# tlemane/kmtricks

Hardware: AMD Instinct MI355X
Metric: k-mers merged/s (merge stage, sum over partitions of input records / time) (higher is better)
Workload: dtype u64 keys / u32 counts (integer)

## Files before the change

### include/kmx.h

```cpp
#ifndef KMX_H
#define KMX_H

#include <stddef.h>
#include <stdint.h>

#ifdef __cplusplus
extern "C" {
#endif

#define KMX_VERSION 2

enum {
  KMX_OK = 0,
  KMX_E_NODEVICE = -1,
  KMX_E_INVAL    = -2,
  KMX_E_NOMEM    = -3,
  KMX_E_HIP      = -4,
  KMX_E_UNSUPPORTED = -5
};

enum {
  KMX_MODE_COUNT = 0,
  KMX_MODE_PA    = 1,
  KMX_MODE_BF    = 2,
  KMX_MODE_BFC   = 3,
  KMX_MODE_BFT   = 4
};

typedef struct kmx_ctx kmx_ctx;

int  kmx_version(void);
int  kmx_device_count(void);
int  kmx_device_memory(int device, uint64_t* free_bytes, uint64_t* total_bytes);
uint64_t kmx_device_warm(int device, uint64_t bytes, const volatile int* stop );
int  kmx_create(int device, kmx_ctx** out);
void kmx_destroy(kmx_ctx* ctx);
const char* kmx_last_error(const kmx_ctx* ctx);
int  kmx_set_profiling(kmx_ctx* ctx, int on);
int  kmx_set_file_order(kmx_ctx* ctx, int on);
void* kmx_stream(kmx_ctx* ctx);


typedef struct {
  const void* recs;
  uint64_t    n;
} kmx_list;

typedef struct {
  uint32_t        n_lists;
  uint32_t        key_words;
  const kmx_list* lists;
  const uint32_t* soft_min;
  uint32_t        rec_min;
  uint32_t        share_min;
  uint32_t        mode;
  uint32_t        bitw;
  uint64_t        lower, upper;
  uint64_t        rows_hint;
  const uint8_t*  list_on_device;
} kmx_merge_task;

#define KMX_STATS_ROWS 6

typedef struct kmx_merge_result kmx_merge_result;

int kmx_merge_dev(kmx_ctx* ctx, const kmx_merge_task* tasks, uint32_t n_tasks, kmx_merge_result** out);
int      kmx_result_wait(kmx_merge_result* r);
double   kmx_result_kernel_ms(kmx_merge_result* r);
int      kmx_result_kernel_parts_ms(kmx_merge_result* r, double* first_ms, double* second_ms);
const char* kmx_result_kernel(const kmx_merge_result* r);
double   kmx_result_transpose_ms(kmx_merge_result* r);
const void* kmx_result_body_dev(kmx_merge_result* r, uint32_t task);
int kmx_result_prepare_body(kmx_merge_result* r, uint32_t task);
uint64_t kmx_result_rows(const kmx_merge_result* r, uint32_t task);
uint64_t kmx_result_sparse_rows(const kmx_merge_result* r, uint32_t task);
uint64_t kmx_result_row_bytes(const kmx_merge_result* r, uint32_t task);
uint64_t kmx_result_body_bytes(const kmx_merge_result* r, uint32_t task);
uint64_t kmx_result_algo_bytes(const kmx_merge_result* r, uint32_t task);
int kmx_result_copy_body(kmx_merge_result* r, uint32_t task, void* host_dst, uint64_t dst_bytes);
int kmx_result_arena(kmx_merge_result* r, uint32_t task, const void** dev_arena, uint64_t* arena_rows);
int kmx_result_copy_order(kmx_merge_result* r, uint32_t task, uint32_t* host_order);
int kmx_result_copy_body_dev(kmx_merge_result* r, uint32_t task, void* dev_dst, uint64_t dst_bytes);
int kmx_result_copy_stats(kmx_merge_result* r, uint32_t task, uint64_t* host_stats );
void kmx_result_free(kmx_merge_result* r);

int kmx_merge_host(kmx_ctx* ctx, const kmx_merge_task* tasks, uint32_t n_tasks, kmx_merge_result** out);
void* kmx_alloc_pinned(size_t bytes);
void  kmx_free_pinned(void* p);

int kmx_merge(kmx_ctx* ctx, const kmx_merge_task* task, void** body, uint64_t* body_bytes,
              uint64_t* rows, uint64_t* stats);


#define KMX_FILTER_M 1u
#define KMX_FILTER_V 2u
#define KMX_FILTER_K 4u
typedef struct {
  uint32_t    key_words;
  uint32_t    mode;
  uint32_t    n_cols;
  uint32_t    want;
  const void* rows;
  uint64_t    n_rows;
  kmx_list    key;
  uint8_t*    marks;
  uint32_t    key_on_device;
} kmx_filter_task;

typedef struct kmx_filter_result kmx_filter_result;

uint8_t* kmx_filter_marks_alloc(kmx_ctx* ctx, uint64_t n);
void     kmx_filter_marks_free(kmx_ctx* ctx, uint8_t* marks);

int kmx_filter_dev(kmx_ctx* ctx, const kmx_filter_task* task, kmx_filter_result** out);
int kmx_filter_host(kmx_ctx* ctx, const kmx_filter_task* task, kmx_filter_result** out);
int      kmx_filter_result_wait(kmx_filter_result* r);
uint64_t kmx_filter_result_rows(kmx_filter_result* r);
uint64_t kmx_filter_result_row_bytes(const kmx_filter_result* r);
uint64_t kmx_filter_result_body_bytes(kmx_filter_result* r);
const void* kmx_filter_result_body_dev(kmx_filter_result* r);
int      kmx_filter_result_copy_body(kmx_filter_result* r, void* host_dst, uint64_t dst_bytes);
uint64_t kmx_filter_result_vector_len(const kmx_filter_result* r);
const void* kmx_filter_result_vector_dev(kmx_filter_result* r);
int      kmx_filter_result_copy_vector(kmx_filter_result* r, uint32_t* host_dst, uint64_t dst_entries);
uint64_t kmx_filter_result_absent(kmx_filter_result* r);
const void* kmx_filter_result_absent_dev(kmx_filter_result* r);
int      kmx_filter_result_copy_absent(kmx_filter_result* r, void* host_dst, uint64_t dst_bytes);
double   kmx_filter_result_kernel_ms(kmx_filter_result* r);
uint64_t kmx_filter_result_algo_bytes(kmx_filter_result* r);
void     kmx_filter_result_free(kmx_filter_result* r);


#define KMX_COMBINE_DROP_LAST 1u
#define KMX_COMBINE_MAX_BLOCKS 64u
typedef struct {
  const void* rows;
  uint64_t    n_rows;
  uint32_t    n_cols;
  uint32_t    count_bytes;
} kmx_block;
typedef struct {
  uint32_t key_words, mode, n_blocks, flags;
  const kmx_block* blocks;
  const uint8_t*   block_on_device;
} kmx_combine_task;

typedef struct kmx_combine_result kmx_combine_result;

int kmx_combine_dev(kmx_ctx* ctx, const kmx_combine_task* task, kmx_combine_result** out);
int kmx_combine_host(kmx_ctx* ctx, const kmx_combine_task* task, kmx_combine_result** out);
int      kmx_combine_result_wait(kmx_combine_result* r);
uint64_t kmx_combine_result_rows(kmx_combine_result* r);
uint64_t kmx_combine_result_row_bytes(const kmx_combine_result* r);
uint64_t kmx_combine_result_body_bytes(kmx_combine_result* r);
const void* kmx_combine_result_body_dev(kmx_combine_result* r);
int      kmx_combine_result_copy_body(kmx_combine_result* r, void* host_dst, uint64_t dst_bytes);
double   kmx_combine_result_kernel_ms(kmx_combine_result* r);
uint64_t kmx_combine_result_algo_bytes(kmx_combine_result* r);
void     kmx_combine_result_free(kmx_combine_result* r);


typedef struct {
  const char*     bases;
  const uint64_t* offsets;
  uint64_t        n_seqs;
  uint32_t        kmer_size, minim_size;
  const uint16_t* repart;
  uint32_t        nb_parts;
  uint32_t        n_cols;
  uint64_t        window;
  const uint8_t* const* rows;
  uint32_t*       hits;
} kmx_query_task;

typedef struct kmx_query_result kmx_query_result;

int kmx_query_dev(kmx_ctx* ctx, const kmx_query_task* task, kmx_query_result** out);
int kmx_query_host(kmx_ctx* ctx, const kmx_query_task* task, kmx_query_result** out);
int      kmx_query_result_wait(kmx_query_result* r);
uint64_t kmx_query_result_n_seqs(const kmx_query_result* r);
int      kmx_query_result_copy_kmers(kmx_query_result* r, uint32_t* host_dst, uint64_t dst_entries);
int      kmx_query_result_copy_hits(kmx_query_result* r, uint32_t* host_dst, uint64_t dst_entries);
uint32_t* kmx_query_result_hits_dev(kmx_query_result* r);
double   kmx_query_result_kernel_ms(kmx_query_result* r);
uint64_t kmx_query_result_algo_bytes(kmx_query_result* r);
void     kmx_query_result_free(kmx_query_result* r);


typedef struct {
  const char*     bases;
  const uint64_t* offsets;
  uint64_t        n_seqs;
  uint32_t        kmer_size, minim_size;
  const uint16_t* repart;
  uint32_t        nb_parts;
  uint32_t        n_cols;
  uint32_t        key_words;
  uint32_t        mode;
  const uint64_t* n_rows;
  const uint8_t* const* rows;
  uint32_t*       hits;
  uint64_t*       sums;
  uint32_t        want_sums;
} kmx_kquery_task;

typedef struct kmx_kquery_result kmx_kquery_result;

int kmx_kquery_dev(kmx_ctx* ctx, const kmx_kquery_task* task, kmx_kquery_result** out);
int kmx_kquery_host(kmx_ctx* ctx, const kmx_kquery_task* task, kmx_kquery_result** out);
int      kmx_kquery_result_wait(kmx_kquery_result* r);
uint64_t kmx_kquery_result_n_seqs(const kmx_kquery_result* r);
int      kmx_kquery_result_copy_kmers(kmx_kquery_result* r, uint32_t* host_dst, uint64_t dst_entries);
int      kmx_kquery_result_copy_hits(kmx_kquery_result* r, uint32_t* host_dst, uint64_t dst_entries);
int      kmx_kquery_result_copy_sums(kmx_kquery_result* r, uint64_t* host_dst, uint64_t dst_entries);
uint32_t* kmx_kquery_result_hits_dev(kmx_kquery_result* r);
uint64_t* kmx_kquery_result_sums_dev(kmx_kquery_result* r);
double   kmx_kquery_result_kernel_ms(kmx_kquery_result* r);
uint64_t kmx_kquery_result_algo_bytes(kmx_kquery_result* r);
void     kmx_kquery_result_free(kmx_kquery_result* r);


typedef struct {
// ... 121 lines not shown
```

### kmtricks_amd/csrc/kmx_api.hip

```cpp
#include "kmx_host.hpp"

#include <algorithm>
#include <chrono>
#include <cmath>
#include <sys/mman.h>
#include <unordered_map>
#include <mutex>
#include <cstdlib>
#include <cstring>
#include <memory>

using namespace kmx;

static thread_local std::string g_create_err;

void* kmx_ctx::dalloc(size_t bytes)
{
  if (bytes == 0) bytes = 256;
  if (bytes >= (8u << 20)) { size_t p2 = (size_t)1 << 23; while (p2 * 2 <= bytes) p2 *= 2; const size_t q = p2 >> 3; bytes = (bytes + q - 1) / q * q; }
  int best = -1;
  for (size_t i = 0; i < pool.size(); i++)
    if (!pool[i].used && pool[i].bytes >= bytes && pool[i].bytes <= 2 * bytes + (1u << 20) &&
        (best < 0 || pool[i].bytes < pool[best].bytes)) best = (int)i;
  if (best >= 0) { pool[best].used = true; return pool[best].p; }
// ... 226 lines not shown
  size_t cap = std::max(bytes, chunk_bytes);
  void* p = nullptr;
  const auto t0 = std::chrono::steady_clock::now();
  hipError_t e = hipMalloc(&p, cap);
  if (e != hipSuccess && cap > bytes) { cap = bytes; e = hipMalloc(&p, cap); }
  { static const bool trace = getenv("KMX_TRACE") != nullptr; if (trace) fprintf(stderr, "[kmx alloc] store chunk %zu MB: %.2f ms\n", cap >> 20, std::chrono::duration<double, std::milli>(std::chrono::steady_clock::now() - t0).count()); }
  if (cur >= 0 && cur != device) (void)hipSetDevice(cur);
  if (e != hipSuccess) return nullptr;
  chunks.push_back({(u8*)p, cap, bytes});
  used += bytes;
  return p;
}
void* kmx_store::try_reserve(size_t bytes)
{
  bytes = (bytes + 255) / 256 * 256;
  if (bytes == 0) bytes = 256;
  std::lock_guard<std::mutex> lk(mu);
  start_ahead();
  if (resvs.size() >= 8 || (limit && used + bytes > limit)) return nullptr;
  for (int pass = 0; pass < 2; pass++) {
    for (size_t i = 0; i < chunks.size(); i++) {
      auto& c = chunks[i];
      if (!chunk_reserved(i) && c.cap - c.fill >= bytes) { resvs.push_back({(int)i, c.fill, bytes}); void* p = c.p + c.fill; c.fill += bytes; used += bytes; return p; }
    }
    if (pass) break;
    { Chunk sp; if (take_spare(bytes, sp)) { chunks.push_back(sp); continue; } }
    int cur = -1; (void)hipGetDevice(&cur);
    if (cur != device && hipSetDevice(device) != hipSuccess) return nullptr;
    const size_t cap = std::max(bytes, chunk_bytes);
    void* p = nullptr;
    const hipError_t e = hipMalloc(&p, cap);
    if (cur >= 0 && cur != device) (void)hipSetDevice(cur);
    if (e != hipSuccess) { (void)hipGetLastError(); return nullptr; }
    chunks.push_back({(u8*)p, cap, 0});
  }
  return nullptr;
}
void kmx_store::commit(void* p, size_t used_bytes)
{
  used_bytes = (used_bytes + 255) / 256 * 256;
  std::lock_guard<std::mutex> lk(mu);
  for (size_t j = 0; j < resvs.size(); j++) {
    const Resv r = resvs[j];
    if (chunks[r.chunk].p + r.off != (u8*)p) continue;
    if (used_bytes > r.bytes) used_bytes = r.bytes;
    chunks[r.chunk].fill = r.off + used_bytes;
    used -= r.bytes - used_bytes;
    resvs.erase(resvs.begin() + j);
    return;
  }
}
extern "C" int kmx_store_create(int device, uint64_t limit_bytes, kmx_store** out)
{
  if (!out) return KMX_E_INVAL;
  *out = nullptr;
  int n = 0;
  if (hipGetDeviceCount(&n) != hipSuccess || n <= 0) { g_create_err = "kmx_store_create: no HIP device; libkmx has no CPU fallback"; return KMX_E_NODEVICE; }
  if (device < 0 || device >= n) { g_create_err = "kmx_store_create: device index out of range"; return KMX_E_INVAL; }
  int cur = -1; (void)hipGetDevice(&cur);
  if (hipSetDevice(device) != hipSuccess) { g_create_err = "kmx_store_create: hipSetDevice failed"; return KMX_E_NODEVICE; }
  size_t fr = 0, tot = 0;
  (void)hipMemGetInfo(&fr, &tot);
  if (cur >= 0 && cur != device) (void)hipSetDevice(cur);
  kmx_store* s = new kmx_store();
  s->device = device;
  s->limit = limit_bytes ? (size_t)limit_bytes : (size_t)(tot / 10 * 6);
  s->chunk_bytes = (size_t)256 << 20;
  { const char* e = getenv("KMX_STORE_CHUNK_MB"); if (e && atol(e) >= 16 && atol(e) <= 65536) s->chunk_bytes = (size_t)atol(e) << 20; }
  *out = s;
  return KMX_OK;
}
extern "C" void kmx_store_destroy(kmx_store* s)
{
  if (!s) return;
  int cur = -1; (void)hipGetDevice(&cur);
  (void)hipSetDevice(s->device);
  (void)hipDeviceSynchronize();
  { std::lock_guard<std::mutex> lk(s->mu); s->stop = true; }
  s->cv.notify_all();
  if (s->ahead.joinable()) s->ahead.join();
  for (auto& c : s->spare) (void)hipFree(c.p);
  for (auto& c : s->chunks) (void)hipFree(c.p);
  if (cur >= 0 && cur != s->device) (void)hipSetDevice(cur);
  delete s;
}
namespace {
std::mutex g_peer_mutex;
signed char g_peer[64][64];
}
int kmx_peer_path(int from, int to)
{
  if (from == to) return 1;
  if (from < 0 || to < 0 || from >= 64 || to >= 64) return 0;
  std::lock_guard<std::mutex> lk(g_peer_mutex);
  if (g_peer[from][to] == 0) {
    int can = 0, cur = -1;
    (void)hipGetDevice(&cur);
    signed char st = -1;
    if (hipDeviceCanAccessPeer(&can, from, to) == hipSuccess && can && hipSetDevice(from) == hipSuccess) {
      const hipError_t e = hipDeviceEnablePeerAccess(to, 0);
      if (e == hipSuccess || e == hipErrorPeerAccessAlreadyEnabled) st = 1;
      (void)hipGetLastError();
    }
    if (cur >= 0) (void)hipSetDevice(cur);
    g_peer[from][to] = st;
    if (getenv("KMX_TRACE")) fprintf(stderr, "[kmx] GPU %d -> GPU %d: %s\n", from, to, st == 1 ? "peer access enabled (copies go over xGMI)" : "no peer access (copies are staged through host memory)");
  }
  return g_peer[from][to] == 1 ? 1 : 0;
}
extern "C" int kmx_peer_access(int from_device, int to_device)
{
  int n = 0;
  if (hipGetDeviceCount(&n) != hipSuccess || from_device < 0 || to_device < 0 || from_device >= n || to_device >= n) return KMX_E_INVAL;
  return kmx_peer_path(from_device, to_device);
}
extern "C" uint64_t kmx_store_used(const kmx_store* s) { return s ? s->used : 0; }
extern "C" uint64_t kmx_store_limit(const kmx_store* s) { return s ? s->limit : 0; }
extern "C" int kmx_copy_to_host(kmx_ctx* ctx, void* dst, const void* src, uint64_t bytes)
{
  if (!ctx) return KMX_E_INVAL;
  if (!bytes) return KMX_OK;
  if (!dst || !src) return ctx->fail(KMX_E_INVAL, "kmx_copy_to_host: null pointer");
  KMX_HIP(ctx, hipSetDevice(ctx->device));
  KMX_HIP(ctx, hipMemcpyAsync(dst, src, bytes, hipMemcpyDeviceToHost, ctx->copy));
  KMX_HIP(ctx, hipStreamSynchronize(ctx->copy));
  return KMX_OK;
}

extern "C" int kmx_copy_to_host_async(kmx_ctx* ctx, void* dst, const void* src, uint64_t bytes, uint32_t* ticket)
{
  if (!ctx) return KMX_E_INVAL;
  if (!ticket || (bytes && (!dst || !src))) return ctx->fail(KMX_E_INVAL, "kmx_copy_to_host_async: null pointer");
  int slot = -1;
  for (int i = 0; i < 8; i++) if (!ctx->copy_out[i]) { slot = i; break; }
  if (slot < 0) return ctx->fail(KMX_E_INVAL, "kmx_copy_to_host_async: KMX_COPIES_AHEAD tickets are out already");
  KMX_HIP(ctx, hipSetDevice(ctx->device));
  if (!ctx->copy_ev[slot]) KMX_HIP(ctx, hipEventCreateWithFlags(&ctx->copy_ev[slot], hipEventDisableTiming));
  if (bytes) KMX_HIP(ctx, hipMemcpyAsync(dst, src, bytes, hipMemcpyDeviceToHost, ctx->copy));
  KMX_HIP(ctx, hipEventRecord(ctx->copy_ev[slot], ctx->copy));
  ctx->copy_out[slot] = true;
  *ticket = (uint32_t)slot;
  return KMX_OK;
}
extern "C" int kmx_copy_wait(kmx_ctx* ctx, uint32_t ticket)
{
  if (!ctx) return KMX_E_INVAL;
  if (ticket >= 8 || !ctx->copy_out[ticket]) return ctx->fail(KMX_E_INVAL, "kmx_copy_wait: no such ticket");
  ctx->copy_out[ticket] = false;
  KMX_HIP(ctx, hipEventSynchronize(ctx->copy_ev[ticket]));
  return KMX_OK;
}

extern "C" int kmx_set_profiling(kmx_ctx* ctx, int on) { if (!ctx) return KMX_E_INVAL; ctx->profiling = on != 0; return KMX_OK; }
extern "C" int kmx_set_file_order(kmx_ctx* ctx, int on) { if (!ctx) return KMX_E_INVAL; ctx->file_order = on != 0; return KMX_OK; }

struct TaskHost {
  u32 N = 0, kw = 1, mode = 0, bitw = 0, c = 1, wl = 0, pivot = 0, rt = 0;
  u32 rec_min = 0, share_min = 0, row_bytes = 0, seg_cap = 0;
  u64 lower = 0, upper = 0, total_recs = 0, out_cap_rows = 0, rows_guess = 0;
  u64 arena_rows = 0;
  bool rows_overflow = false;
  std::vector<u32> len;
  size_t o_recs = 0, o_len = 0, o_smin = 0, o_bounds = 0, o_stats = 0, o_ctrl = 0, o_segs = 0;
  u8* d_out = nullptr; size_t out_bytes = 0;
  u16* d_rowrec = nullptr;
  u32 bft_c = 1;
  u8* d_img = nullptr; size_t img_bytes = 0;
  u64 t_rows = 0, t_cols = 0;
  Seg* d_segs = nullptr;
  Seg* d_segs_own = nullptr;
  u64 rows = 0, nsegs = 0;
  bool done = false;
  bool handed_back = false;
  u32 nblk = 0, nb = 0, rt_cols = 0, slots_cap = 0;
  size_t o_skel = 0, o_nskel = 0, o_rbounds = 0;
  u8* d_ov = nullptr;
  size_t o_spdir = 0;
  size_t o_ovx = 0; u32 xcap = 0;
  u64 sparse_rows = 0;
  u8* d_body = nullptr;
  bool body_ready = false;
  hipEvent_t ev_body = nullptr;
  void* d_body_tmp = nullptr;
  u8* d_dense = nullptr; u32 dpitch = 0, dense_cap = 0; size_t o_gbase = 0;
  u8* d_narrow = nullptr; u32 npitch = 0;
  u64 row_keys = 0;
  bool ordered = false;
  std::vector<u32> src;
  int kernel = 0;
};

struct kmx_merge_result {
  kmx_ctx* ctx = nullptr;
  std::vector<TaskHost> tasks;
  u8* d_meta = nullptr; size_t meta_bytes = 0;
  u8* h_meta = nullptr;
  size_t o_tasks = 0, o_items = 0, o_ticket = 0, o_ctrl0 = 0;
  u32 n_items = 0, grid = 0, max_n = 0, max_c = 0;
  int bf_lds = 0;
  bool is_bf = false, is_bft = false, waited = false;
  bool cols_ext = false, slices_full = false;
  bool cols_resc = false;
  bool share_fix = false;
  bool cols_ord = false;
  bool back_other = false;
  bool rows_small = false;
  bool cols_narrow = false;
  bool rerun_rows = false;
  bool pivot_auto = false;
  bool use_pivot = false;
  bool use_cols = false, cols_auto = false, can_pivot = false, auto_sel = false;
  bool divergent = false;
  u32 given = 0;
  std::vector<TaskHost> subs;
  size_t o_subtasks = 0, o_subitems = 0, o_cols = 0, o_citems = 0;
  u32 n_subitems = 0, n_citems = 0, sub_grid = 0, cols_grid = 0, sub_max_c = 0, sub_max_n = 0, items_grid = 0;
  int status = KMX_OK;
  hipEvent_t ev0 = nullptr, ev1 = nullptr;
  hipEvent_t ev_mid = nullptr;
  hipEvent_t ev2 = nullptr;
  u8* d_in = nullptr;
  u64* d_rem = nullptr; u32 rem_cap = 0;
  bool bft_two_walks = false;
  hipEvent_t ev_in = nullptr;
  u64* d_hctrl = nullptr;
  hipEvent_t ev_pre = nullptr;
  hipEvent_t ev_up = nullptr;
  hipEvent_t ev_done = nullptr;
};

static size_t align_up(size_t x, size_t a) { return (x + a - 1) / a * a; }

static u32 cols_row_lists(u32 rec_min)
{
  for (u32 S = std::max<u32>(8, rec_min + 2); S <= 32; S++) {
    const u32 m = S - rec_min + 1;
    double p = 1.0;
    for (u32 i = 0; i < m; i++) p *= (double)(S - i) / (double)(i + 1) * 0.035;
    if (p < 2e-9) return S;
  }
  return 0;
}

__global__ void k_ctrl_mirror(const u64* __restrict__ src, u64* __restrict__ dst, u32 n)
{
  const u32 i = blockIdx.x * blockDim.x + threadIdx.x;
  if (i < n) dst[i] = src[i];
  __threadfence_system();
}
static int mirror_and_mark(kmx_merge_result* R);
__global__ void k_share_fix(const TaskDev* __restrict__ tasks, u32 kw);

static int launch_batch(kmx_merge_result* R, bool with_bounds)
{
  kmx_ctx* ctx = R->ctx;
  const TaskDev* d_tasks = reinterpret_cast<const TaskDev*>(R->d_meta + R->o_tasks);
  const uint2* d_items = reinterpret_cast<const uint2*>(R->d_meta + R->o_items);
  u32* d_ticket = reinterpret_cast<u32*>(R->d_meta + R->o_ticket);
  const int kw = (int)R->tasks[0].kw, mode = (int)R->tasks[0].mode;
  const ColsOps& CO = cols_ops(kw);
  const u32 nt = (u32)R->tasks.size();
  if (!R->use_cols) KMX_HIP(ctx, hipMemsetAsync(d_ticket, 0, 16, ctx->stream));
  if (ctx->profiling && !R->ev0) { KMX_HIP(ctx, hipEventCreate(&R->ev0)); KMX_HIP(ctx, hipEventCreate(&R->ev1)); }
  if (R->is_bf) {
    if (with_bounds && !R->is_bft) KMX_HIP(ctx, launch_range_bounds_bf(d_tasks, nt, R->max_n, R->max_c, ctx->stream));
    if (R->ev0) KMX_HIP(ctx, hipEventRecord(R->ev0, ctx->stream));
    if (R->is_bft) {
      u32 rt_max = 0; bool rec_bits = true, any_share = false;
      for (auto& H : R->tasks) { rt_max = std::max(rt_max, H.rt); rec_bits = rec_bits && std::max(H.rec_min, H.share_min) <= 1u; any_share = any_share || H.share_min > 0; }
      const u32 bgrid = std::min(R->n_items, (u32)ctx->n_cu * 2u);
      static const bool two_walks_env = getenv("KMX_BFT_TWO_WALKS") != nullptr;
      if (rec_bits && any_share && !R->bft_two_walks && !two_walks_env && !R->d_rem) {
        u64 per_tile = 0;
        for (auto& H : R->tasks) { const u64 tiles = std::max<u64>(1, ((H.upper - H.lower + 1) + H.rt - 1) / H.rt); per_tile = std::max(per_tile, H.total_recs / tiles); }
        u64 cap = std::max<u64>(4096, per_tile / 4);
        cap = std::min<u64>(cap, ((1ull << 30) / 8) / std::max(1u, bgrid));
        R->rem_cap = (u32)cap;
        R->d_rem = (u64*)ctx->dalloc((size_t)bgrid * cap * 8);
      }
      const bool one_walk = R->d_rem && !R->bft_two_walks;
      bool wide = false;
      for (auto& H : R->tasks) { const double m = (double)H.total_recs / H.N * (double)H.rt / (double)(H.upper - H.lower + 1); wide = wide || m + 2.6 * std::sqrt(m) + 8 > (double)bft_round_records(false); }
      KMX_HIP(ctx, launch_merge_bft(d_tasks, d_items, R->n_items, d_ticket, bgrid, R->max_n, rt_max, rec_bits, wide, one_walk ? R->d_rem : nullptr, R->rem_cap, ctx->stream));
    } else
    KMX_HIP(ctx, launch_merge_bf(mode == KMX_MODE_BFC, d_tasks, d_items, R->n_items, d_ticket, R->grid, R->bf_lds, ctx->stream));
  } else if (R->use_cols) {
    const TaskDev* d_subs = reinterpret_cast<const TaskDev*>(R->d_meta + R->o_subtasks);
    const uint2* d_subitems = reinterpret_cast<const uint2*>(R->d_meta + R->o_subitems);
    const ColsDev* d_cols = reinterpret_cast<const ColsDev*>(R->d_meta + R->o_cols);
    const uint2* d_citems = reinterpret_cast<const uint2*>(R->d_meta + R->o_citems);
    static const bool overlap = getenv("KMX_COLS_PREP_OVERLAP") != nullptr;
    hipStream_t ps = overlap ? ctx->aux : ctx->stream;
    if (!R->ev_pre) KMX_HIP(ctx, hipEventCreateWithFlags(&R->ev_pre, hipEventDisableTiming));
    if (overlap && ctx->stream_shared) {
      KMX_HIP(ctx, hipEventRecord(R->ev_pre, ctx->stream));
      KMX_HIP(ctx, hipStreamWaitEvent(ctx->aux, R->ev_pre, 0));
    }
    if (!overlap) KMX_HIP(ctx, hipStreamWaitEvent(ctx->stream, R->ev_up, 0));
    KMX_HIP(ctx, launch_range_bounds(kw, d_subs, nt, R->sub_max_n, R->sub_max_c, ps));
    KMX_HIP(ctx, CO.skel(d_subs, d_subitems, R->n_subitems, ps));
    KMX_HIP(ctx, CO.prep(d_tasks, d_subs, d_cols, nt, ps));
    KMX_HIP(ctx, hipEventRecord(R->ev_pre, ps));
    KMX_HIP(ctx, hipStreamWaitEvent(ctx->stream, R->ev_up, 0));
    KMX_HIP(ctx, launch_range_bounds(kw, d_tasks, nt, R->max_n, R->max_c, ctx->stream));
    KMX_HIP(ctx, hipStreamWaitEvent(ctx->stream, R->ev_pre, 0));
    if (R->ev0) KMX_HIP(ctx, hipEventRecord(R->ev0, ctx->stream));
    const u32 cols_grid_env = getenv("KMX_COLS_GRID") ? (u32)atoi(getenv("KMX_COLS_GRID")) : 0u;
    const u32 sparse_cus_env = getenv("KMX_SPARSE_CUS") ? (u32)atoi(getenv("KMX_SPARSE_CUS")) : 0u;
    KMX_HIP(ctx, CO.merge(mode, (R->cols_ext ? 1 : 0) | (R->cols_resc ? 2 : 0) | (R->cols_ord ? 4 : 0) | (R->cols_narrow ? 8 : 0), d_tasks, d_cols, d_citems, R->n_citems, d_ticket,
                          cols_grid_env ? std::min(cols_grid_env, R->cols_grid) : R->cols_grid, ctx->stream));
    if (R->ev0) { if (!R->ev_mid) KMX_HIP(ctx, hipEventCreate(&R->ev_mid)); KMX_HIP(ctx, hipEventRecord(R->ev_mid, ctx->stream)); }
    KMX_HIP(ctx, CO.sparse(mode | (R->cols_resc ? 2 : 0) | (R->cols_ord ? 4 : 0), d_tasks, d_cols, d_items, R->n_items, nt, d_ticket, sparse_cus_env ? std::min(sparse_cus_env, (u32)ctx->n_cu) : (u32)ctx->n_cu, ctx->stream));
    if (R->share_fix) {
      if ((size_t)R->max_n * 4 > 48 * 1024) KMX_HIP(ctx, hipFuncSetAttribute(reinterpret_cast<const void*>(&k_share_fix), hipFuncAttributeMaxDynamicSharedMemorySize, (int)std::min<size_t>((size_t)R->max_n * 4, 160 * 1024)));
      hipLaunchKernelGGL(k_share_fix, dim3((unsigned)ctx->n_cu * 2u, nt), dim3(256), (size_t)R->max_n * 4, ctx->stream, (const TaskDev*)d_tasks, kw);
      KMX_HIP(ctx, hipGetLastError());
    }
    if (R->ev0) KMX_HIP(ctx, hipEventRecord(R->ev1, ctx->stream));
    return mirror_and_mark(R);
  } else {
    if (with_bounds) KMX_HIP(ctx, launch_range_bounds(kw, d_tasks, nt, R->max_n, R->max_c, ctx->stream));
    if (R->ev0) KMX_HIP(ctx, hipEventRecord(R->ev0, ctx->stream));
    if (R->use_pivot) KMX_HIP(ctx, launch_merge_pivot(kw, mode, d_tasks, d_items, R->n_items, d_ticket, R->grid, ctx->stream));
    else if (R->rows_small) KMX_HIP(ctx, launch_merge_rows_s(kw, mode, d_tasks, d_items, R->n_items, d_ticket, R->grid, R->max_n, ctx->stream));
    else KMX_HIP(ctx, launch_merge_rows(kw, mode, d_tasks, d_items, R->n_items, d_ticket, R->grid, R->max_n, ctx->stream));
  }
  if (R->ev0) KMX_HIP(ctx, hipEventRecord(R->ev1, ctx->stream));
  return mirror_and_mark(R);
}

__global__ __launch_bounds__(256)
void k_share_fix(const TaskDev* __restrict__ tasks, u32 kw)
{
  extern __shared__ u32 sm_s[];
  const TaskDev& T = tasks[blockIdx.y];
  if (T.mode != KMX_MODE_COUNT || T.share_min <= max(1u, T.rec_min)) return;
  if (T.ctrl[2] & (u64)(ERR_FALLBACK | ERR_ROWS_OVERFLOW)) return;
  const u64 rows = T.ctrl[0];
  const u32 lane = threadIdx.x & 63u, N = T.N;
  for (u32 l = threadIdx.x; l < N; l += 256) sm_s[l] = T.soft_min[l];
  __syncthreads();
  const u64 nw = (u64)gridDim.x * 4u;
  for (u64 r = (u64)blockIdx.x * 4u + (threadIdx.x >> 6); r < rows; r += nw) {
    u32* const cnt = reinterpret_cast<u32*>(T.out + r * T.row_bytes + 8u * kw);
    u32 solid = 0, weak = 0;
    for (u32 l0 = 0; l0 < N; l0 += 64u * 16u) {
      u32 c[16];
#pragma unroll
      for (int j = 0; j < 16; j++) { const u32 l = l0 + 64u * j + lane; c[j] = l < N ? cnt[l] : 0u; }
#pragma unroll
      for (int j = 0; j < 16; j++) { const u32 l = l0 + 64u * j + lane; if (c[j]) { if (c[j] >= sm_s[l]) solid++; else weak++; } }
    }
#pragma unroll
    for (int o = 32; o > 0; o >>= 1) { solid += (u32)__shfl_xor((int)solid, o); weak += (u32)__shfl_xor((int)weak, o); }
    if (solid >= T.share_min || !weak) continue;
    for (u32 l = lane; l < N; l += 64) {
      const u32 c = cnt[l];
      if (c && c < sm_s[l]) {
        cnt[l] = 0;
        atomicAdd(reinterpret_cast<unsigned long long*>(&T.stats[(u64)N + l]), ~0ULL);
        atomicAdd(reinterpret_cast<unsigned long long*>(&T.stats[5ull * N + l]), 0ULL - (unsigned long long)c);
      }
    }
  }
}

static int mirror_and_mark(kmx_merge_result* R)
{
  kmx_ctx* ctx = R->ctx;
  if (!R->d_hctrl) {
    void* dp = nullptr;
    KMX_HIP(ctx, hipHostGetDevicePointer(&dp, R->h_meta + R->o_ctrl0, 0));
    R->d_hctrl = reinterpret_cast<u64*>(dp);
  }
  const u32 n = (u32)R->tasks.size() * 8;
  hipLaunchKernelGGL(k_ctrl_mirror, dim3((n + 255) / 256), dim3(256), 0, ctx->stream,
                     reinterpret_cast<const u64*>(R->d_meta + R->o_ctrl0), R->d_hctrl, n);
  KMX_HIP(ctx, hipGetLastError());
  if (!R->ev_done) KMX_HIP(ctx, hipEventCreateWithFlags(&R->ev_done, hipEventDisableTiming));
  KMX_HIP(ctx, hipEventRecord(R->ev_done, ctx->stream));
  return KMX_OK;
}

extern "C" int kmx_merge_dev(kmx_ctx* ctx, const kmx_merge_task* tasks, uint32_t n_tasks, kmx_merge_result** out)
{
  if (!ctx) return KMX_E_INVAL;
  if (!tasks || !n_tasks || !out) return ctx->fail(KMX_E_INVAL, "kmx_merge_dev: null argument");
  *out = nullptr;
  KMX_HIP(ctx, hipSetDevice(ctx->device));
  const u32 kw = tasks[0].key_words, mode = tasks[0].mode;
  if (kw < 1 || kw > 4) return ctx->fail(KMX_E_INVAL, "key_words must be 1 ... 4");
  if (mode > KMX_MODE_BFT) return ctx->fail(KMX_E_INVAL, "unknown mode");
  const bool is_bft = mode == KMX_MODE_BFT;
  const bool is_bf = mode == KMX_MODE_BF || mode == KMX_MODE_BFC || is_bft;
  const ColsOps& CO = cols_ops((int)kw);
  if (is_bf && kw != 1) return ctx->fail(KMX_E_INVAL, "BF/BFC modes take hash keys (key_words = 1)");

  std::unique_ptr<kmx_merge_result> R(new kmx_merge_result());
  R->ctx = ctx; R->is_bf = is_bf; R->is_bft = is_bft;
  R->tasks.resize(n_tasks);
  u64 grand_total = 0;
  {
    u32 mxn0 = 0; for (u32 t = 0; t < n_tasks; t++) mxn0 = std::max(mxn0, tasks[t].n_lists);
    const char* e = getenv("KMX_ROWS_SMALL");
    R->rows_small = !is_bf && kw <= 2 && mxn0 <= 256 && !(e && e[0] == '0');
  }
  const bool rsm = R->rows_small;
  for (u32 t = 0; t < n_tasks; t++) {
    const kmx_merge_task& K = tasks[t];
    TaskHost& H = R->tasks[t];
    if (K.key_words != kw || K.mode != mode) return ctx->fail(KMX_E_INVAL, "all tasks of a batch must share key_words and mode");
    if (K.n_lists == 0 || !K.lists || !K.soft_min) return ctx->fail(KMX_E_INVAL, "task without lists / soft_min");
    H.N = K.n_lists; H.kw = kw; H.mode = mode; H.bitw = K.bitw;
    H.rec_min = K.rec_min; H.share_min = K.share_min; H.lower = K.lower; H.upper = K.upper;
    if (!is_bf && H.N > (u32)rows_cap((int)kw, ~0u)) return ctx->fail(KMX_E_UNSUPPORTED, "more than " + std::to_string(rows_cap((int)kw, ~0u)) + " lists per merge task (COUNT/PA) not supported yet");
    H.len.resize(H.N);
    u32 pivot = 0;
    for (u32 i = 0; i < H.N; i++) {
      if (K.lists[i].n > 0xFFFFFFF0ULL) return ctx->fail(KMX_E_UNSUPPORTED, "list longer than 2^32 records");
      if (K.lists[i].n && !K.lists[i].recs) return ctx->fail(KMX_E_INVAL, "null record pointer");
      if (((uintptr_t)K.lists[i].recs) & 3u) return ctx->fail(KMX_E_INVAL, "record pointers must be 4-byte aligned");
      H.len[i] = (u32)K.lists[i].n;
      H.total_recs += K.lists[i].n;
      if (H.len[i] > H.len[pivot]) pivot = i;
    }
    const u32 longest = H.len[pivot];
    if (H.N >= 5) {
      u32 cand[5] = {0, H.N / 4, H.N / 2, (3 * H.N) / 4, H.N - 1};
      std::sort(cand, cand + 5, [&](u32 a, u32 b) { return H.len[a] < H.len[b]; });
      if (H.len[cand[2]] > 0) pivot = cand[2];
    }
    H.pivot = pivot;
    grand_total += H.total_recs;
    if (is_bf) {
      if (K.upper < K.lower) return ctx->fail(KMX_E_INVAL, "BF window upper < lower");
      if (mode == KMX_MODE_BFC && (K.bitw == 0 || K.bitw > 32)) return ctx->fail(KMX_E_INVAL, "bitw must be in 1..32");
      H.row_bytes = mode != KMX_MODE_BFC ? (H.N + 7) / 8 : (u32)(((u64)H.N * K.bitw + 7) / 8);
      u32 rt = (40960u / H.row_bytes) & ~63u; if (rt < 64) rt = 64;
      if (!is_bft && (u64)rt * H.row_bytes > 96 * 1024) return ctx->fail(KMX_E_UNSUPPORTED, "BF row too wide for one LDS tile");
      H.rt = is_bft ? bft_tile_rows(K.rec_min, K.share_min) : rt;
      H.out_bytes = (size_t)((K.upper - K.lower + 1) * H.row_bytes);
      if (is_bft && H.N > bft_max_lists()) return ctx->fail(KMX_E_UNSUPPORTED, "more than " + std::to_string(bft_max_lists()) + " samples per hash:bft task not supported");
      if (is_bft) {
        H.t_rows = (K.upper - K.lower + 1 + 7) & ~7ULL; H.t_cols = (u64)H.row_bytes * 8;
        H.img_bytes = 0;
        H.nblk = (u32)((H.t_cols + bft_block_lists() - 1) / bft_block_lists());
        H.out_bytes = (size_t)(H.t_cols * (H.t_rows >> 3));
      }
    } else {
      H.row_bytes = kw * 8 + (mode == KMX_MODE_COUNT ? 4 * H.N : (H.N + 7) / 8);
      u32 wl = 0; while (wl < 6 && (H.N << (wl + 1)) <= (u32)(rsm ? rows_s_cap((int)kw, H.N) : rows_cap((int)kw, H.N))) wl++;
      H.wl = wl;
      if (H.row_bytes > (rsm ? rows_s_image_bytes((int)kw) : rows_image_bytes((int)kw))) return ctx->fail(KMX_E_UNSUPPORTED, "row wider than the LDS row image");
      u64 guess = K.rows_hint ? K.rows_hint : 2ULL * longest + 4096;
      if (ctx->rows_per_longest > 0.0) guess = std::max<u64>(guess, (u64)(ctx->rows_per_longest * 1.125 * (double)longest) + 4096);
      if (guess > H.total_recs) guess = H.total_recs;
      H.rows_guess = std::max<u64>(guess, 1);
    }
  }
  if (is_bft) {
    bool all1 = true; u64 wsum = 0;
    for (auto& H : R->tasks) { all1 = all1 && std::max(H.rec_min, H.share_min) <= 1u; wsum += H.upper - H.lower + 1; }
    u32 mxn = 0; for (auto& H : R->tasks) mxn = std::max(mxn, H.N);
// ... 2030 lines not shown
```

### kmtricks_amd/csrc/kmx_host.hpp

```cpp
#pragma once
#include <hip/hip_runtime.h>
#include <string>
#include <functional>
#include <vector>
#include "kmx_dev.hpp"
#include "skf.hpp"
#include "../../include/kmx.h"

namespace kmx {

int rows_lds_bytes(int kw, u32 n_lists);
int rows_cap(int kw, u32 n_lists);
int rows_wgs_per_cu(int kw);
u32 rows_chunk_rows(u32 row_bytes);
u32 rows_image_bytes(int kw);
hipError_t launch_range_bounds(int kw, const TaskDev* tasks, u32 n_tasks, u32 max_n, u32 max_c, hipStream_t st);
hipError_t launch_merge_rows(int kw, int mode, const TaskDev* tasks, const uint2* items, u32 n_items, u32* ticket,
                             u32 grid_x, u32 max_n, hipStream_t st);
int rows_s_cap(int kw, u32 n_lists);
int rows_s_wgs_per_cu(int kw);
u32 rows_s_image_bytes(int kw);
hipError_t launch_merge_rows_s(int kw, int mode, const TaskDev* tasks, const uint2* items, u32 n_items, u32* ticket, u32 grid_x, u32 max_n, hipStream_t st);
int pivot_lds_bytes(int kw);
u32 pivot_max_lists();
hipError_t launch_merge_pivot(int kw, int mode, const TaskDev* tasks, const uint2* items, u32 n_items, u32* ticket,
                              u32 grid_x, hipStream_t st);
struct ColsOps {
  int (*lds_bytes)();
  u32 (*block_lists)();
  u32 (*wgs_per_cu)();
  u32 (*tile_rows)(u32 nb);
  u64 (*scratch_keys)(u32 slots, u32 nblk);
  u64 (*scratch_counts)(u32 slots, u32 nblk);
  u64 (*ext_entries)(u32 slots, u32 nblk);
  u32 (*skel_cap)();
  hipError_t (*skel)(const TaskDev* subs, const uint2* items, u32 n_items, hipStream_t st);
  hipError_t (*prep)(const TaskDev* tasks, const TaskDev* subs, const ColsDev* cols, u32 n_tasks, hipStream_t st);
  hipError_t (*merge)(int mode, int ext, const TaskDev* tasks, const ColsDev* cols, const uint2* items, u32 n_items, u32* ticket, u32 grid_x, hipStream_t st);
  hipError_t (*sparse)(int mode, const TaskDev* tasks, const ColsDev* cols, const uint2* range_items, u32 n_items, u32 n_tasks, u32* ticket, u32 n_cu, hipStream_t st);
  u64 (*dir_bytes)(u32 slots);
  u32 (*groups)(u32 slots);
  hipError_t (*offsets)(const ColsDev* cols, u32 task, u64* goff, hipStream_t st);
  hipError_t (*gather)(const TaskDev* tasks, const ColsDev* cols, u32 task, u32 n_groups, const u64* goff, u8* body, hipStream_t st);
  hipError_t (*order)(const TaskDev* tasks, const ColsDev* cols, u32 task, u32 n_groups, const u64* goff, u32* order, hipStream_t st);
  void (*dbg_dump)();
  void (*phase_prof_dump)();
  u32 key_words;
};
const ColsOps& cols_ops_k1();
const ColsOps& cols_ops_k2();
inline const ColsOps& cols_ops(int kw) { return kw == 2 ? cols_ops_k2() : cols_ops_k1(); }
int bf_lds_bytes(u32 rt, u32 nb, u32 n_lists);
hipError_t launch_range_bounds_bf(const TaskDev* tasks, u32 n_tasks, u32 max_n, u32 max_c, hipStream_t st);
hipError_t launch_merge_bf(int bfc, const TaskDev* tasks, const uint2* items, u32 n_items, u32* ticket,
                           u32 grid_x, int lds, hipStream_t st);
u32 bft_tile_rows(u32 rec_min, u32 share_min);
u32 bft_block_lists();
u32 bft_max_lists();
u32 bft_round_records(bool wide);
u32 bft_fit_rows(u32 max_n, bool bits);
hipError_t launch_merge_bft(const TaskDev* tasks, const uint2* items, u32 n_items, u32* ticket, u32 grid_x, u32 max_n, u32 rt_max, bool rec_bits, bool wide, u64* rem, u32 rem_cap, hipStream_t st);
hipError_t launch_bit_transpose(const u8* in, u8* out, u64 nrows, u64 ncols, hipStream_t st);
u32 filter_tiles(u32 n);
hipError_t launch_filter_match(int kw, const u8* rows, u32 n_rows, u64 irb, const u8* key, u32 n_key, int pa,
                               u32* hit, u32* vec, u8* marks, u32* tile_cnt, hipStream_t st);
hipError_t launch_filter_scan(u32* a, u32 n, hipStream_t st);
hipError_t launch_filter_move(const u8* rows, u32 n_rows, u64 irb, u64 orb, const u32* hit, const u32* vec, const u32* tile_base,
                              u8* out, hipStream_t st);
hipError_t launch_filter_absent_count(const u8* marks, u32 n_key, u32* tile_cnt, hipStream_t st);
hipError_t launch_filter_absent_scatter(int kw, const u8* key, const u8* marks, u32 n_key, const u32* tile_base, u8* out, hipStream_t st);
struct CombineBlock {
  const u8* rows;
  u64 irb;
  u64 key_off;
  u32 n_rows, n_cols;
  u32 cb;
  u32 pos;
  u32 toff;
  u32 ntiles;
};
u32 combine_tiles(u32 n);
hipError_t launch_combine_keys(int kw, const CombineBlock* blocks, u32 nb, u32 n_slots, u64* keys, hipStream_t st);
hipError_t launch_combine_first(int kw, const CombineBlock* blocks, u32 nb, u32 n_slots, const u64* keys, u32* tcnt, u64* fbits, hipStream_t st);
hipError_t launch_combine_scan(const CombineBlock* blocks, u32 nb, u32* tcnt, hipStream_t st);
hipError_t launch_combine_place(int kw, const CombineBlock* blocks, u32 nb, u32 n_slots, const u64* keys, u32* tcnt, u64* fbits, u32* src, u64 cap, hipStream_t st);
hipError_t launch_combine_total(const CombineBlock* blocks, u32 nb, const u32* tcnt, const u32* src, u64 cap, int drop_last, u32* tot, hipStream_t st);
hipError_t launch_combine_move(int pa, const CombineBlock* blocks, u32 nb, u32 kb, u32 n_cols, u32 orb, const u32* src, u64 cap, const u32* tot,
                               u8* out, hipStream_t st);
void query_chunks(u64 n_bases, u32 n_parts, u32* n_tiles, u32* n_chunks, u32* tiles_per_chunk);
hipError_t launch_query_keys(int kw, const char* bases, const u64* offsets, u32 n_seqs, u64 n_bases, int k, int m, const u16* repart, u64 window,
                             u32 n_tiles, u32 n_chunks, u32 tiles_per_chunk, u64* keys, u32* hist , u32* n_kmers , hipStream_t st);
hipError_t launch_query_parts(const u32* cell, u32 n_parts, u32 n_chunks, u32* pstart , hipStream_t st);
hipError_t launch_query_scatter(const u64* keys, const u64* offsets, u32 n_seqs, u64 n_bases, u32 n_tiles, u32 n_chunks, u32 tiles_per_chunk,
                                u32* cell, u64* recs, hipStream_t st);
hipError_t launch_query_gather(const u64* recs, u64 rec_bound, const u32* pstart, u32 n_parts, const u8* const* rows, u32 nb, u32 n_cols,
                               u32* hits, u32 n_cu, hipStream_t st);
hipError_t launch_query_gather_keyed(const u64* recs, u64 rec_bound, const u32* pstart, u32 n_parts, const u8* const* rows, u64 stride, u32 skip,
                                     u32 nb, u32 n_cols, u32* hits, u32 n_cu, hipStream_t st);
hipError_t launch_kquery_keys(int kw, const char* bases, const u64* offsets, u32 n_seqs, u64 n_bases, int k, int m, const u16* repart,
                              u32 n_tiles, u32 n_chunks, u32 tiles_per_chunk, u16* parts , u64* words ,
                              u32* hist , u32* n_kmers , hipStream_t st);
hipError_t launch_kquery_scatter(const u16* parts, const u64* offsets, u32 n_seqs, u64 n_bases, u32 n_tiles, u32 n_chunks, u32 tiles_per_chunk,
                                 u32* cell, u64* recs, hipStream_t st);
hipError_t launch_kquery_search(int kw, u64* recs, u64 rec_bound, const u32* pstart, u32 n_parts, const u8* const* rows, const u32* n_rows,
                                u64 stride, const u64* words, u64 n_bases, u32* n_found , u32 n_cu, hipStream_t st);
hipError_t launch_kquery_gather(const u64* recs, u64 rec_bound, const u32* pstart, u32 n_parts, const u8* const* rows, u64 stride, u32 skip,
                                u32 n_cols, u32* hits, u64* sums , u32 n_cu, hipStream_t st);

hipError_t launch_zquery_scatter(const u64* keys, u64 n_bases, u32 n_tiles, u32 n_chunks, u32 tiles_per_chunk, u32* cell, u64* recs ,
                                 hipStream_t st);
hipError_t launch_zquery_rows(const u64* recs, u64 rec_bound, const u32* pstart, u32 n_parts, const u8* const* rows, u32 nb, u32 n_cols,
                              u8* bits , u32 n_cu, hipStream_t st);
hipError_t launch_zquery_window(const u64* keys, const u64* offsets, u32 n_seqs, u64 n_bases, u32 z, const u8* bits, u32 nb, u32 n_cols,
                                u32* n_kmers , u32* hits, u32 n_cu, hipStream_t st);
}

struct kmx_count_req { kmx::u32 k; int hash_mode; kmx::u64 window; kmx::u32 hard_min; uint64_t** keys; uint32_t** counts; uint64_t* n_out;
                       kmx_store* const* stores = nullptr; kmx::u32 n_stores = 0; kmx_list* lists = nullptr;
                       kmx::u32 inner_parts = 0; };
int kmx_count_from_device(kmx_ctx* ctx, const kmx::u8* d_recs, const kmx::u64* d_prefix, const kmx::u16* d_part, kmx::u32 n_recs,
                          kmx::u64 total_kmers, kmx::u32 n_parts, const kmx::u64* part_kmer_off , const kmx_count_req& rq,
                          const kmx::u32* d_sbase = nullptr );
void kmx_launch_pack_bases(const char* d_bases, kmx::u64 n, kmx::u64* out , hipStream_t st);
struct kmx_fast_split {
  const kmx::u64* d_words;
  const kmx::u32* d_sbase;
  const kmx::u64* d_boff;
  const kmx::u16* d_part16;
  const kmx::u32* d_blk;
  kmx::SkfCtl* d_ctl;
  const uint4* d_parts;
  const kmx::u32* d_cfirst;
  kmx::u32* d_cnt;
  kmx::u32* d_sflags;
  kmx::u32 n_parts; kmx::u64 kmer_bound; kmx::u32 tb_max, nc_max, nb_max;
  kmx::SkfCtl* h_ctl;
  const uint4* h_parts;
  unsigned long long* d_strand;
  std::function<int()> behind_scatter;
  std::function<int()> before_wait;
  kmx::u32* d_koff; kmx::u32* h_koff; size_t back_bytes;
};
kmx::SkfLayout kmx_fast_layout(int key_words );
int kmx_count_fast_tail(kmx_ctx* ctx, const kmx_fast_split& F, const kmx_count_req& rq);
void kmx_phase_mark(int i);
void kmx_count_chain_begin(kmx_ctx* ctx);
void kmx_count_chain_end(kmx_ctx* ctx);
void kmx_count_chain_forget(kmx_ctx* ctx);

int kmx_peer_path(int from, int to);
void* kmx_pinned_alloc(size_t bytes);
bool kmx_is_pinned(const void* p, size_t n);
void kmx_pinned_free(void* p);

struct kmx_pool_block { void* p; size_t bytes; bool used; };

#include <mutex>
#include <thread>
#include <condition_variable>
struct kmx_store {
  int device = 0;
  size_t limit = 0, used = 0, chunk_bytes = 0;
  struct Chunk { kmx::u8* p; size_t cap, fill; };
  std::vector<Chunk> chunks;
  std::mutex mu;
  void* alloc(size_t bytes);
  struct Resv { int chunk; size_t off, bytes; };
  std::vector<Resv> resvs;
  bool chunk_reserved(size_t i) const { for (auto& r : resvs) if (r.chunk == (int)i) return true; return false; }
  std::vector<Chunk> spare; std::thread ahead; std::condition_variable cv; bool stop = false, ahead_on = false;
  void start_ahead();
  bool take_spare(size_t bytes, Chunk& out);
  void* try_reserve(size_t bytes);
  void commit(void* p, size_t used_bytes);
};

struct kmx_ctx {
  int device = 0;
  hipStream_t stream = nullptr;
  bool stream_shared = false;
  hipStream_t copy = nullptr;
  hipStream_t up = nullptr;
  hipEvent_t copy_ev[8] = {}; bool copy_out[8] = {};
  struct ReadsAhead { char* d = nullptr; size_t bytes = 0; hipEvent_t ev = nullptr; bool live = false; };
  ReadsAhead ahead[4];
  hipStream_t aux = nullptr;
  hipEvent_t ev_chain = nullptr;
  hipEvent_t ev_split = nullptr;
  int n_cu = 0;
  std::string err;
  bool profiling = false;
  std::vector<kmx_pool_block> pool;
  size_t big_max = 0;
  std::vector<kmx_pool_block> hpool;
  unsigned pivot_backoff = 0, pivot_skip = 0;
  unsigned cols_backoff = 0, cols_skip = 0;
  bool cols_min_env = false;
  unsigned cols_min_lists = 192, cols_min_lists_ord = 257;
// ... 42 lines not shown
```

### kmtricks_amd/csrc/merge_cols.hip

```cpp
#include "kmx_host.hpp"
#include <algorithm>
#include <cstdio>
#include <cstring>

#ifndef KMX_CL_KW
#define KMX_CL_KW 1
#endif
#if KMX_CL_KW == 1
#define CLNS cols_k1
#elif KMX_CL_KW == 2
#define CLNS cols_k2
#elif KMX_CL_KW == 3
#define CLNS cols_k3
#else
#define CLNS cols_k4
#endif

namespace kmx { namespace CLNS {

#ifndef KMX_CL_TPB
#define KMX_CL_TPB 1024
#endif
constexpr int CL_TPB = KMX_CL_TPB;
constexpr int CL_WGS = 1024 / CL_TPB;
#ifndef KMX_CL_G
#define KMX_CL_G 8
#endif
constexpr int CL_G = KMX_CL_G;
constexpr int KW = KMX_CL_KW;
constexpr int RB = KW * 8 + 4;
constexpr int RD = RB / 4;
constexpr int EW = KW + 1;
constexpr int CL_U = KW == 1 ? 16 : 8;
constexpr int CL_W = CL_G * CL_U;
constexpr int CL_NB = CL_TPB / CL_G;
constexpr int CL_IMG = 61440 / CL_WGS;
constexpr int CL_RT = CL_W * 7 / 8;
constexpr int CL_KPL = (CL_RT + 63) / 64;
constexpr int CL_NT = (CL_KPL == 1 && CL_WGS == 1 && KW == 1) ? 2 : 1;
constexpr int CL_PT = CL_KPL == 1 ? 2048 : 4096;
constexpr int CL_PTSHIFT = CL_PT == 2048 ? 21 : 20;
constexpr int CL_HALVES = CL_KPL;
constexpr int CL_SEEDS = 256;
constexpr int CL_OVW = 128;
constexpr int CL_XS = 3 * CL_OVW;
constexpr int CL_NW = CL_TPB / 64;
constexpr int CK_BITS = 1 << 17;
constexpr int CP_MAXSEG = 2048;

__device__ u32 kmx_cols_dbg[16];

namespace {

typedef u32 u32x3 __attribute__((ext_vector_type(3), aligned(4)));
typedef u32 u32x4 __attribute__((ext_vector_type(4), aligned(4)));
typedef __attribute__((address_space(1))) const u32x3 gu32x3;
typedef __attribute__((address_space(1))) const u32x4 gu32x4;
typedef __attribute__((address_space(1))) u64 gu64w;
typedef u64 u64x2 __attribute__((ext_vector_type(2), aligned(8)));
__device__ __forceinline__ u32 cl_uni(u32 v) { return (u32)__builtin_amdgcn_readfirstlane((int)v); }
__device__ __forceinline__ u64 cl_uni64(u64 v) { return (u64)cl_uni((u32)v) | ((u64)cl_uni((u32)(v >> 32)) << 32); }

#if KMX_CL_KW == 1
typedef u64 CKey;
struct CRec { u32x3 v; };
struct ClEnt { u32 klo, khi, idx, pad; };
__device__ __forceinline__ bool ck_lt(CKey a, CKey b) { return a < b; }
__device__ __forceinline__ bool ck_eq(CKey a, CKey b) { return a == b; }
__device__ __forceinline__ CKey ck_inf() { return ~0ULL; }
__device__ __forceinline__ u64 ck_fold(CKey k) { return k; }
__device__ __forceinline__ CKey ck_uni(CKey k) { return cl_uni64(k); }
__device__ __forceinline__ CKey ck_load(const u8* p) { return load_key<1>(p).w[0]; }
__device__ __forceinline__ void ck_store(u32* p, CKey k) { p[0] = (u32)k; p[1] = (u32)(k >> 32); }
__device__ __forceinline__ CKey cl_key(const CRec& r) { return (u64)r.v.x | ((u64)r.v.y << 32); }
__device__ __forceinline__ u32 cl_cnt(const CRec& r) { return r.v.z; }
__device__ __forceinline__ CRec cl_none() { CRec r; r.v.x = ~0u; r.v.y = ~0u; r.v.z = 0; return r; }
__device__ __forceinline__ CRec cl_load(gu32* p) { CRec r; r.v = *(gu32x3*)p; return r; }
__device__ __forceinline__ bool ent_hit(const ClEnt& e, CKey k) { return (((u64)e.khi << 32) | e.klo) == k && e.idx != 0; }
__device__ __forceinline__ void ent_set(ClEnt& e, CKey k) { e.klo = (u32)k; e.khi = (u32)(k >> 32); }
__device__ __forceinline__ ClEnt ent_load(const ClEnt* tab, u32 h) { const uint4 v = reinterpret_cast<const uint4*>(tab)[h]; ClEnt e; e.klo = v.x; e.khi = v.y; e.idx = v.z; e.pad = v.w; return e; }
#else
struct CKey { u64 lo, hi; };
struct CRec { u32x4 k; u32 c; };
struct ClEnt { u64 lo, hi; u32 idx, pad[3]; };
__device__ __forceinline__ bool ck_lt(CKey a, CKey b) { return a.hi != b.hi ? a.hi < b.hi : a.lo < b.lo; }
__device__ __forceinline__ bool ck_eq(CKey a, CKey b) { return a.lo == b.lo && a.hi == b.hi; }
__device__ __forceinline__ CKey ck_inf() { CKey k; k.lo = ~0ULL; k.hi = ~0ULL; return k; }
__device__ __forceinline__ u64 ck_fold(CKey k) { const u64 h = k.hi * 0x9E3779B97F4A7C15ULL; return k.lo ^ h ^ (h >> 29); }
__device__ __forceinline__ CKey ck_uni(CKey k) { CKey r; r.lo = cl_uni64(k.lo); r.hi = cl_uni64(k.hi); return r; }
__device__ __forceinline__ CKey ck_load(const u8* p) { const Key<2> k = load_key<2>(p); CKey r; r.lo = k.w[0]; r.hi = k.w[1]; return r; }
__device__ __forceinline__ void ck_store(u32* p, CKey k) { p[0] = (u32)k.lo; p[1] = (u32)(k.lo >> 32); p[2] = (u32)k.hi; p[3] = (u32)(k.hi >> 32); }
__device__ __forceinline__ CKey cl_key(const CRec& r) { CKey k; k.lo = (u64)r.k.x | ((u64)r.k.y << 32); k.hi = (u64)r.k.z | ((u64)r.k.w << 32); return k; }
__device__ __forceinline__ u32 cl_cnt(const CRec& r) { return r.c; }
__device__ __forceinline__ CRec cl_none() { CRec r; r.k.x = ~0u; r.k.y = ~0u; r.k.z = ~0u; r.k.w = ~0u; r.c = 0; return r; }
__device__ __forceinline__ CRec cl_load(gu32* p) { CRec r; r.k = *(gu32x4*)p; r.c = p[4]; return r; }
__device__ __forceinline__ bool ent_hit(const ClEnt& e, CKey k) { return e.lo == k.lo && e.hi == k.hi && e.idx != 0; }
__device__ __forceinline__ void ent_set(ClEnt& e, CKey k) { e.lo = k.lo; e.hi = k.hi; }
__device__ __forceinline__ ClEnt ent_load(const ClEnt* tab, u32 h)
{
  const uint4 v = reinterpret_cast<const uint4*>(tab)[2 * h]; const u32 ix = reinterpret_cast<const u32*>(tab)[8 * h + 4];
  ClEnt e; e.lo = (u64)v.x | ((u64)v.y << 32); e.hi = (u64)v.z | ((u64)v.w << 32); e.idx = ix; return e;
}
#endif
__device__ __forceinline__ bool ck_le(CKey a, CKey b) { return !ck_lt(b, a); }
__device__ __forceinline__ void cl_barrier() { asm volatile("s_waitcnt lgkmcnt(0)\n\ts_barrier" ::: "memory"); }
__device__ __forceinline__ u32 cl_thash(CKey key, u32 hf)
{
  const u64 k = ck_fold(key);
  if (hf & 0x80000000u) {
    const u64 m = 0x9E3779B97F4A7C15ULL + 2ULL * (u64)(hf & 0xFFFFu) * 0xBF58476D1CE4E5B9ULL;
    return (u32)((k * m) >> (CL_PT == 2048 ? 53 : 52));
  }
#if KMX_CL_KW == 1
  const u32 x = ((u32)k ^ (u32)(k >> (hf >> 24))) & 0xFFFFFFu;
#else
  const u32 f = (u32)k ^ (u32)(k >> 32);
  const u32 x = (f ^ (f >> 8)) & 0xFFFFFFu;
#endif
  return ((u32)__umul24(x, hf) >> CL_PTSHIFT) & (u32)(CL_PT - 1);
}
__device__ __forceinline__ u32 cl_mult(u32 seed)
{
  if (KW == 2 && seed >= 16u) return 0x80000000u | (seed - 15u);
  if (seed >= 64u) return 0x80000000u | (seed - 63u);
  return ((0x9E3779u + seed * 0x5A6B2u) & 0xFFFFFFu) | ((13u + (seed * 7u) % 19u) << 24);
}
__device__ __forceinline__ u32 cl_mix(CKey key)
{
  const u64 k = ck_fold(key);
  u32 x = (u32)k ^ ((u32)(k >> 32) * 0x9E3779B1u);
  x *= 0x85EBCA6Bu; x ^= x >> 15; x *= 0x2C1B3C6Du; x ^= x >> 13;
  return x;
}
__device__ __forceinline__ u32 cl_build(ClEnt* tab, const CKey (&key)[CL_KPL], const bool (&have)[CL_KPL], u32 lane, u32 (&slot)[CL_KPL])
{
  for (u32 s = 0; s < (u32)CL_SEEDS; s++) {
    const u32 mult = cl_mult(s);
    u32 h[CL_KPL], old[CL_KPL];
    bool clash = false;
#pragma unroll
    for (int x = 0; x < CL_KPL; x++) {
      h[x] = cl_thash(key[x], mult);
      old[x] = have[x] ? atomicCAS(&tab[h[x]].idx, 0u, lane + 64u * x + 1) : 0u;
      clash |= old[x] != 0;
    }
    if (__ballot(clash) == 0) {
#pragma unroll
      for (int x = 0; x < CL_KPL; x++) { if (have[x]) ent_set(tab[h[x]], key[x]); slot[x] = h[x]; }
      return mult;
    }
#pragma unroll
    for (int x = 0; x < CL_KPL; x++) if (have[x] && old[x] == 0) atomicExch(&tab[h[x]].idx, 0u);
  }
  return 0;
}

}

#ifndef KMX_SK_TPB
#define KMX_SK_TPB 256
#endif
constexpr int SK_TPB = KMX_SK_TPB;
constexpr int SK_CAP = 2048;

__global__ __launch_bounds__(SK_TPB)
void k_cols_skel(const TaskDev* __restrict__ subs, const uint2* __restrict__ items, u32 n_items)
{
  __shared__ CKey ks[SK_CAP];
  __shared__ u32 wsum[SK_TPB / 64];
  const u32 item = blockIdx.x;
  if (item >= n_items) return;
  const TaskDev& S = subs[items[item].x];
  const u32 range = items[item].y, N = S.N, rec_min = max(1u, S.rec_min);
  const u32 tid = threadIdx.x, lane = tid & 63, wave = tid >> 6;
  u32 total = 0;
  for (u32 i = 0; i < N; i++) total += S.bounds[(u64)(range + 1) * N + i] - S.bounds[(u64)range * N + i];
  Seg sg; sg.range = range; sg.seq = 0; sg.row_off = (u64)range * SK_CAP; sg.nrows = 0; sg.pad = 0;
  if (total > (u32)SK_CAP) {
    if (tid == 0) { atomicOr(&S.ctrl[2], (u64)ERR_ROWS_OVERFLOW); S.segs[range] = sg; atomicAdd(&S.ctrl[1], 1ULL); }
    return;
  }
  __shared__ u32 irregular;
  u32 maxn = 1;
  for (u32 i = 0; i < N; i++) maxn = max(maxn, S.bounds[(u64)(range + 1) * N + i] - S.bounds[(u64)range * N + i]);
  u32 L = 1; while (L < maxn) L <<= 1;
  u32 SP = 1; while (SP < N) SP <<= 1;
  const bool runs = (u64)SP * L <= (u64)SK_CAP;
  u32 P = 2;
  if (runs) P = max(2u, SP * L); else while (P < total) P <<= 1;
  if (tid == 0) irregular = 0;
  if (runs) for (u32 t = tid; t < P; t += SK_TPB) ks[t] = ck_inf();
  __syncthreads();
  {
    const u32 tpl = max(1u, (u32)SK_TPB / N);
    for (u32 i = tid / tpl; i < N; i += (u32)SK_TPB / tpl) {
      u32 off = 0;
      if (!runs) for (u32 j = 0; j < i; j++) off += S.bounds[(u64)(range + 1) * N + j] - S.bounds[(u64)range * N + j];
      const u32 lo = S.bounds[(u64)range * N + i], n = S.bounds[(u64)(range + 1) * N + i] - lo, smin = S.soft_min[i];
      const u8* base = S.recs[i] + (u64)lo * RB;
      for (u32 e = tid % tpl; e < n; e += tpl) {
        const u32* rp = reinterpret_cast<const u32*>(base + (u64)e * RB);
        const bool solid = rp[RD - 1] >= smin;
        const CKey key = solid ? ck_load(reinterpret_cast<const u8*>(rp)) : ck_inf();
        if (!runs) ks[off + e] = key;
        else { ks[i * L + ((i & 1u) ? L - 1 - e : e)] = key; if (!solid) irregular = 1; }
      }
    }
  }
  if (!runs) for (u32 t = total + tid; t < P; t += SK_TPB) ks[t] = ck_inf();
  __syncthreads();
  const u32 k0 = (runs && !irregular) ? 2 * L : 2;
  for (u32 k = k0; k <= P; k <<= 1) {
    for (u32 j = k >> 1; j > 0; j >>= 1) {
      for (u32 t = tid; t < P / 2; t += SK_TPB) {
        const u32 a = ((t & ~(j - 1)) << 1) | (t & (j - 1)), b = a | j;
        const CKey x = ks[a], y = ks[b];
        const bool up = (a & k) == 0;
        if (ck_lt(y, x) == up) { ks[a] = y; ks[b] = x; }
      }
      __syncthreads();
    }
  }
  const u32 per = P / SK_TPB ? P / SK_TPB : 1;
  u32 mine = 0, keptm = 0, nsolid = 0, ncov = 0;
  for (u32 x = 0; x < per; x++) {
    const u32 i = tid * per + x;
    if (i < P) {
      const CKey k = ks[i];
      const bool real = !ck_eq(k, ck_inf());
      const bool kept = real && (i == 0 || !ck_eq(ks[i - 1], k)) && i + rec_min - 1 < P && ck_eq(ks[i + rec_min - 1], k);
      keptm |= (kept ? 1u : 0u) << x; mine += kept ? 1u : 0u;
      if (real && (range & 7u) == 0) {
        nsolid++;
        bool cov = false;
        for (u32 j = 0; j < rec_min && !cov; j++) cov = i >= j && i - j + rec_min - 1 < P && ck_eq(ks[i - j], k) && ck_eq(ks[i - j + rec_min - 1], k);
        ncov += cov ? 1u : 0u;
      }
    }
  }
  if ((range & 7u) == 0) {
#pragma unroll
    for (int off = 32; off > 0; off >>= 1) { nsolid += __shfl_xor(nsolid, off); ncov += __shfl_xor(ncov, off); }
    if (lane == 0 && nsolid) { atomicAdd(&S.ctrl[4], (u64)nsolid); atomicAdd(&S.ctrl[5], (u64)ncov); }
  }
  const u32 incl = wave_incl_scan(mine, (int)lane);
  if (lane == 63) wsum[wave] = incl;
  __syncthreads();
  u32 base = incl - mine, nk = 0;
  for (u32 w = 0; w < SK_TPB / 64; w++) { if (w < wave) base += wsum[w]; nk += wsum[w]; }
  CKey* out = reinterpret_cast<CKey*>(S.out) + (u64)range * SK_CAP;
  for (u32 x = 0; x < per; x++) if ((keptm >> x) & 1u) out[base++] = ks[tid * per + x];
  if (tid == 0) { sg.nrows = nk; S.segs[range] = sg; atomicAdd(&S.ctrl[1], 1ULL); atomicAdd(&S.ctrl[3], (u64)nk); }
}

constexpr int CP_TPB = 1024;
__global__ __launch_bounds__(CP_TPB)
void k_cols_prep(const TaskDev* __restrict__ tasks, const TaskDev* __restrict__ subs, const ColsDev* __restrict__ cols)
{
  const TaskDev& T = tasks[blockIdx.x];
  const TaskDev& S = subs[blockIdx.x];
  const ColsDev& C = cols[blockIdx.x];
  __shared__ u32 s_off[CP_MAXSEG];
  __shared__ u64 s_ord[CP_MAXSEG];
  __shared__ u32 s_n[CP_MAXSEG];
  const u32 tid = threadIdx.x;
  const u64 serr = S.ctrl[2], nseg64 = S.ctrl[1], rows = S.ctrl[3];
  if (tid == 0) T.ctrl[7] = rows;
  const u64 slots = rows / C.rt + T.c + 2;
  const bool dense_small = C.dense != nullptr && rows > (u64)C.dense_cap;
  const bool bad = serr != 0 || nseg64 > (u64)CP_MAXSEG || nseg64 > S.seg_cap || rows > T.out_cap_rows || rows > 0xFFFFFF00ULL ||
                   slots > C.slots_cap || dense_small;
  const u64 nsolid = S.ctrl[4], ncov = S.ctrl[5];
  const bool divergent = (nsolid - ncov) * 8 > nsolid;
  if (divergent && !bad) {
    if (tid == 0) { atomicOr(&T.ctrl[2], (u64)(ERR_FALLBACK | ERR_DIVERGENT)); *C.nskel = 0; atomicAdd(&kmx_cols_dbg[4], 1u); }
    for (u32 j = tid; j <= T.c; j += CP_TPB) { C.rbounds[j] = 0; if (C.gbase) C.gbase[j] = 0; }
    return;
  }
  if (bad) {
    const bool only_dense = dense_small && !(serr != 0 || nseg64 > (u64)CP_MAXSEG || nseg64 > S.seg_cap || rows > T.out_cap_rows || rows > 0xFFFFFF00ULL || slots > C.slots_cap);
    if (tid == 0) { atomicOr(&T.ctrl[2], (u64)(ERR_FALLBACK | (only_dense ? ERR_DENSE_CAP : 0))); *C.nskel = 0; }
    for (u32 j = tid; j <= T.c; j += CP_TPB) { C.rbounds[j] = 0; if (C.gbase) C.gbase[j] = 0; }
    return;
  }
  const u32 nseg = (u32)nseg64;
  const u32 srb = S.row_bytes;
  for (u32 i = tid; i < nseg; i += CP_TPB) { const Seg a = S.segs[i]; s_ord[i] = ((u64)a.range << 32) | a.seq; s_n[i] = a.nrows; }
  __syncthreads();
  for (u32 i = tid; i < nseg; i += CP_TPB) {
    const u64 mine = s_ord[i];
    u32 off = 0;
    for (u32 j = 0; j < nseg; j++) off += s_ord[j] < mine ? s_n[j] : 0u;
    s_off[i] = off;
  }
  __syncthreads();
  for (u32 i = tid >> 6; i < nseg; i += CP_TPB / 64) {
    const Seg a = S.segs[i];
    const u8* src = S.out + a.row_off * srb;
    for (u32 r = tid & 63u; r < a.nrows; r += 64) reinterpret_cast<CKey*>(C.skel)[(u64)s_off[i] + r] = ck_load(src + (u64)r * srb);
  }
  __syncthreads();
  const u32 np = T.len[T.pivot];
  for (u32 j = tid; j <= T.c; j += CP_TPB) {
    u32 res;
    if (j == 0) res = 0;
    else if (j == T.c) res = (u32)rows;
    else {
      const u32 pos = (u32)(((u64)j * np) / T.c);
      const CKey q = ck_load(T.recs[T.pivot] + (u64)pos * RB);
      u32 lo = 0, hi = (u32)rows;
      while (lo < hi) { const u32 mid = lo + ((hi - lo) >> 1); if (ck_lt(reinterpret_cast<const CKey*>(C.skel)[mid], q)) lo = mid + 1; else hi = mid; }
      res = lo;
    }
    C.rbounds[j] = res;
  }
  if (tid == 0) {
    *C.nskel = (u32)rows;
    T.ctrl[0] = rows; T.ctrl[1] = 1; T.ctrl[3] = rows;
    Seg sg; sg.range = 0; sg.seq = 0; sg.row_off = 0; sg.nrows = (u32)rows; sg.pad = 0;
    T.segs[0] = sg;
  }
  if (C.gbase) {
    __shared__ u32 s_ng;
    __syncthreads();
    if (tid == 0) {
      u32 g = 0;
      for (u32 j = 0; j < T.c; j++) { C.gbase[j] = g; const u32 n = C.rbounds[j + 1] - C.rbounds[j]; g += max(1u, (n + C.rt - 1) / C.rt) * (u32)CL_HALVES; }
      C.gbase[T.c] = g; s_ng = g;
      atomicMax(C.gmax, g);
    }
    __syncthreads();
    const u32 ng = s_ng;
    for (u32 g = tid; g < ng; g += CP_TPB) {
      u32 lo = 0, hi = T.c;
      while (hi - lo > 1) { const u32 mid = (lo + hi) >> 1; if (C.gbase[mid] <= g) lo = mid; else hi = mid; }
      C.gmap[g] = make_uint4(lo + 1, g - C.gbase[lo], C.rbounds[lo], C.rbounds[lo + 1]);
    }
  }
}

__device__ const u32 kmx_cols_sentinel[8] = {~0u, ~0u, KW == 1 ? 0u : ~0u, KW == 1 ? 0u : ~0u, 0u, 0u, 0u, 0u};

#ifdef KMX_PHASE_PROF
__device__ u64 kmx_cols_prof[8];
__device__ u64 kmx_sparse_prof[8];
#ifndef KMX_PROF_TID
#define KMX_PROF_TID 512
#endif
#endif

constexpr u64 CL_NONSOLID = 1ULL << 63;
template <int MODE, bool EXT, bool RESC, bool ORD, bool NAR>
__global__ __launch_bounds__(CL_TPB, CL_WGS)
void k_merge_cols(const TaskDev* __restrict__ tasks, const ColsDev* __restrict__ cols, const uint2* __restrict__ items,
                  u32 n_items, u32* ticket)
{
  extern __shared__ __attribute__((aligned(16))) unsigned char smem[];
  u32* const img = reinterpret_cast<u32*>(smem);
  ClEnt* const ptab = reinterpret_cast<ClEnt*>(smem + CL_IMG);
  u32* const sh = reinterpret_cast<u32*>(smem + CL_IMG + CL_NT * CL_PT * sizeof(ClEnt));
  const u32 dummy = (u32)(CL_IMG + CL_NT * CL_PT * sizeof(ClEnt)) / 4 + 16 + (u32)(threadIdx.x & 63);

  const int tid = threadIdx.x, lane = tid & 63;
  const u32 wave = cl_uni((u32)tid >> 6);
  for (int t = tid; t < CL_IMG / 16; t += CL_TPB) reinterpret_cast<uint4*>(img)[t] = make_uint4(0, 0, 0, 0);
  for (int t = tid; t < CL_NT * CL_PT; t += CL_TPB) ptab[t].idx = 0;
  if (tid == 0) { sh[1] = 0; sh[2] = 0; sh[3] = 0; }
#ifdef KMX_PHASE_PROF
  long long pt[8] = {0, 0, 0, 0, 0, 0, 0, 0}; long long pc = clock64();
#define CLPH(i) do { const long long n_ = clock64(); pt[i] += n_ - pc; pc = n_; } while (0)
#else
#define CLPH(i) do {} while (0)
#endif

  for (;;) {
    if (tid == 0) sh[0] = atomicAdd(ticket, 1u);
    __syncthreads();
    const u32 item = cl_uni(sh[0]);
    __syncthreads();
    if (item >= n_items) {
#ifdef KMX_PHASE_PROF
      if (tid == KMX_PROF_TID) for (int i = 0; i < 8; i++) atomicAdd(&kmx_cols_prof[i], (u64)pt[i]);
#endif
      return;
    }
    const TaskDev& T = tasks[items[item].x];
    const ColsDev& C = cols[items[item].x];
    if (__syncthreads_or((__hip_atomic_load(&T.ctrl[2], __ATOMIC_RELAXED, __HIP_MEMORY_SCOPE_AGENT) & (u64)(ERR_FALLBACK | ERR_ROWS_OVERFLOW)) != 0)) continue;
    const u32 N = cl_uni(T.N), row_bytes = cl_uni(T.row_bytes), nblk = cl_uni(C.nblk), nbs = cl_uni(C.nb), rt = cl_uni(C.rt);
    const u32 range = cl_uni(items[item].y) / nblk, blk = cl_uni(items[item].y) - range * nblk;
    const u32 col0 = blk * nbs, nbl = min(nbs, N - col0);
    const u32 iw = MODE == 0 ? nbs : (nbs + 31) / 32;
    const u32 s_lo = cl_uni(C.rbounds[range]), s_hi = cl_uni(C.rbounds[range + 1]);
    const u32 ntiles = max(1u, (s_hi - s_lo + rt - 1) / rt);
    const u32 slot0 = s_lo / rt + range;
    const CKey* const skel = reinterpret_cast<const CKey*>(C.skel);
    constexpr bool ord = ORD;
    u8* const obase = ord ? C.dense : T.out + KW * 8;
    const u32 opitch = ord ? cl_uni(C.dpitch) : row_bytes;
    static_assert(!NAR || (MODE == 0 && ORD), "the byte-wide side store is for count rows in file order");
    u8* const nar = NAR ? C.dnarrow : nullptr;
    const u32 npitch = NAR ? cl_uni(C.npitch) : 0u;
    u8* const img8 = reinterpret_cast<u8*>(img);
    u8* const rowbig = reinterpret_cast<u8*>(smem) + CL_RT * CL_NB;
    const u32 dummyb = dummy * 4u;

    const u32 lg = (u32)tid / CL_G, r = (u32)tid & (CL_G - 1);
    const bool on = lg < nbl;
    const u32 li = col0 + (on ? lg : 0u);
    u32 cur = on ? T.bounds[(u64)range * N + li] : 0u;
    const u32 end = on ? T.bounds[(u64)(range + 1) * N + li] : 0u;
    const u32 smin = T.soft_min[li];
    gu32* const base = (gu32*)(uintptr_t)T.recs[li];
    gu32* const sentinel = (gu32*)(uintptr_t)kmx_cols_sentinel;
    CRec rec[CL_U];
#pragma unroll
    for (int u = 0; u < CL_U; u++) {
      const u32 ix = cur + ((r + CL_G * u - cur) & (CL_W - 1));
      rec[u] = cl_none();
      if (ix < end) rec[u] = cl_load(base + (u64)ix * RD);
    }
    u64 tsum = 0; u32 tn = 0;
    u64 rsum = 0; u32 rn = 0;
    const bool rescue = RESC && cl_uni(T.share_min) != 0;
    CKey skn[CL_KPL];
    u32 myslot[CL_KPL];
    bool failed = false;
#pragma unroll
    for (int x = 0; x < CL_KPL; x++) { skn[x] = ck_inf(); myslot[x] = 0; }
    if (tid < 64) {
      bool have[CL_KPL];
#pragma unroll
      for (int x = 0; x < CL_KPL; x++) {
        const u32 j = (u32)tid + 64u * x;
        have[x] = j < rt && s_lo + j < s_hi;
        if (have[x]) {
          skn[x] = skel[s_lo + j];
          if (blk == 0 && !ord) ck_store(reinterpret_cast<u32*>(T.out + (u64)(s_lo + j) * row_bytes), skn[x]);
        }
      }
      const u32 mult = cl_build(ptab, skn, have, (u32)tid, myslot);
      if (tid == 0) { sh[4] = mult; if (mult == 0) { failed = true; atomicAdd(&kmx_cols_dbg[0], 1u); } }
    }
    CKey khi_n = ntiles > 1 ? skel[s_lo + rt] : ck_inf();
    CKey kmid_n = (CL_HALVES > 1 && s_lo + 56 < s_hi) ? skel[s_lo + 56] : ck_inf();
    u32 rnd = 0;
    cl_barrier();
    CLPH(0);

    for (u32 q = 0; q < ntiles; q++) {
      const u32 s0 = s_lo + q * rt;
      const u32 rte = min(rt, s_hi - s0);
      const bool last = cl_uni(q + 1 == ntiles ? 1u : 0u) != 0;
      const CKey khi = ck_uni(khi_n);
      const CKey kmid = ck_uni(kmid_n);
      if (!last) {
        if (tid < 64) {
#pragma unroll
          for (int x = 0; x < CL_KPL; x++) { const u32 j = (u32)tid + 64u * x; skn[x] = ck_inf(); if (j < rt && s0 + rt + j < s_hi) skn[x] = skel[s0 + rt + j]; }
        }
        khi_n = q + 2 < ntiles ? skel[s0 + 2 * rt] : ck_inf();
        kmid_n = (CL_HALVES > 1 && s0 + rt + 56 < s_hi) ? skel[s0 + rt + 56] : ck_inf();
      }
      const ClEnt* const tab = ptab + (q % CL_NT) * CL_PT;
      const u32 mult = cl_uni(sh[4 + (q % CL_NT)]);
      gu64w* const ovk0 = (gu64w*)(uintptr_t)(C.ovkeys + (((((u64)(slot0 + q) * CL_HALVES) * nblk + blk) * CL_NW + wave) * CL_OVW) * EW);
      gu64w* const ovk1 = ovk0 + (u64)nblk * CL_NW * CL_OVW * EW;
      const u64 li_hi = (u64)li << 32;
      u32 wov = 0, wov1 = 0;
      u32 xb0 = 0, xb1 = 0;
      auto extend = [&](u32& xb) {
        u32 b = 0;
        if (lane == 0) b = atomicAdd(C.xcur, (u32)CL_XS);
        b = cl_uni(b);
        xb = (b + (u32)CL_XS <= C.xcap) ? b + 1u : 0xFFFFFFFFu;
      };
      gu64w* const ovx = (gu64w*)(uintptr_t)C.ovx;

      for (;;) {
        if (tid == 0) sh[1 + (rnd == 2 ? 0 : rnd + 1)] = 0;
        u32 consm = 0;
        if (last) {
#pragma unroll
          for (int u = 0; u < CL_U; u++) consm |= ((cur + ((r + CL_G * u - cur) & (CL_W - 1))) < end ? 1u : 0u) << u;
        } else {
#pragma unroll
          for (int u = 0; u < CL_U; u++) consm |= (ck_lt(cl_key(rec[u]), khi) ? 1u : 0u) << u;
        }
        asm volatile("" : "+v"(consm));
#if KMX_CL_KW == 1
#pragma unroll
        for (int x = 0; x < CL_KPL; x++) asm volatile("" : "+v"(skn[x]));
#endif
        CLPH(1);
#pragma unroll
        for (int g = 0; g < CL_U; g += 4) {
          __builtin_amdgcn_sched_barrier(0);
          u32 curg = cur; asm volatile("" : "+v"(curg));
          ClEnt pe[4];
#pragma unroll
          for (int j = 0; j < 4; j++) pe[j] = ent_load(tab, cl_thash(cl_key(rec[g + j]), mult));
          u32 ovm = 0;
#pragma unroll
          for (int j = 0; j < 4; j++) {
            const int u = g + j;
            const bool cons = (consm >> u) & 1u;
            const CKey k = cl_key(rec[u]);
            const u32 c = cl_cnt(rec[u]);
            const bool solid = cons && c >= smin;
            const bool hit = ent_hit(pe[j], k);
            tsum += solid ? c : 0u;
            tn += (cons && !solid) ? 1u : 0u;
            const bool dep = RESC ? (cons && hit && (solid || rescue)) : (solid && hit);
            if (RESC) { const bool rs = cons && hit && !solid && rescue; rsum += rs ? c : 0u; rn += rs ? 1u : 0u; }
            bool big = false;
            if (NAR) { img8[dep ? __umul24(pe[j].idx - 1, nbs) + lg : dummyb] = (u8)min(c, 255u); big = dep && c > 254u; }
            else if (MODE == 0) img[dep ? __umul24(pe[j].idx - 1, iw) + lg : dummy] = c;
            else if (dep) atomicOr(&img[__umul24(pe[j].idx - 1, iw) + (lg >> 5)], 1u << (lg & 31u));
            ovm |= (((RESC ? cons : solid) && !hit) ? 1u : 0u) << j;
            if (NAR) ovm |= (big ? 0x11u : 0u) << j;
          }
          asm volatile("" : "+v"(tsum), "+v"(tn));
          if (RESC) asm volatile("" : "+v"(rsum), "+v"(rn));
#pragma unroll
          for (int j = 0; j < 4; j++) {
            u64 bal = __ballot((ovm >> j) & 1u);
            if (bal) {
              if (NAR) {
                const bool isbig = (ovm >> (4 + j)) & 1u;
                if (__builtin_expect(__ballot(isbig) != 0, 0)) {
                  if (isbig) { const u32 rw = ent_load(tab, cl_thash(cl_key(rec[g + j]), mult)).idx - 1; reinterpret_cast<u32*>(C.dense + (u64)(s0 + rw) * opitch)[li] = cl_cnt(rec[g + j]); rowbig[rw] = 1; }
                  ovm &= isbig ? ~(1u << j) : ~0u;
                  bal = __ballot((ovm >> j) & 1u);
                }
              }
              const CKey kk = cl_key(rec[g + j]);
              const u64 pay = li_hi | cl_cnt(rec[g + j]) | ((RESC && cl_cnt(rec[g + j]) < smin) ? CL_NONSOLID : 0ULL);
#if KMX_CL_KW == 1
#define CL_PUT(o, pos) do { (o)[2 * (pos)] = kk; (o)[2 * (pos) + 1] = pay; } while (0)
#else
// ... 916 lines not shown
    if (s_base == ~0ULL) { hand_back(12); return false; }
    auto count_rows = [&]() { if (tid == 0 && nks) { atomicAdd(&T.ctrl[0], (u64)nks); atomicAdd(&T.ctrl[3], (u64)nks); atomicAdd(&T.ctrl[6], (u64)nks); } };
    const u64 base = s_base;
    if (base + grows > T.out_cap_rows) { if (tid == 0) atomicOr(&T.ctrl[2], (u64)ERR_ROWS_OVERFLOW); count_rows(); return true; }
    if (npass == 1) write_pass(base, nks, 0, dn, true);
    else {
      u64 b = base;
      for (u32 p = 0; p < npass; p++) {
        const u32 dlo = (u32)(((u64)dn * p) / npass), dhi = (u32)(((u64)dn * (p + 1)) / npass);
        const u32 nk = sort_pass(p, true, dlo, dhi - dlo);
        __syncthreads();
        write_pass(b, nk, dlo, dhi - dlo, false);
        b += nk + (dhi - dlo);
      }
    }
    count_rows();
    return true;
  };

  if (!ORD) {
    const u32 item = blockIdx.x;
    if (item < n_items) {
      const TaskDev& T = tasks[items[item].x];
      const ColsDev& C = cols[items[item].x];
      if (!__syncthreads_or((__hip_atomic_load(&T.ctrl[2], __ATOMIC_RELAXED, __HIP_MEMORY_SCOPE_AGENT) & (u64)(ERR_FALLBACK | ERR_ROWS_OVERFLOW)) != 0)) {
        const u32 range = items[item].y, rt = C.rt;
        const u32 s_lo = C.rbounds[range], s_hi = C.rbounds[range + 1];
        const u32 ngroups = max(1u, (s_hi - s_lo + rt - 1) / rt) * CL_HALVES;
        for (u32 q = blockIdx.y; q < ngroups; q += CK_Z) if (!group(T, C, range, q, s_lo, s_hi, 0u)) break;
      }
    }
  } else {
    for (;;) {
      __syncthreads();
      if (tid == 0) s_tk = atomicAdd(&tkt[1], 1u);
      __syncthreads();
      const u32 t = s_tk;
      const u32 ti = t % n_tasks, g = t / n_tasks;
      if (g >= tkt[2] || g >= tkt[3]) {
        if (g < tkt[2] && tid == 0) atomicAdd(&kmx_cols_dbg[9], 1u);
        break;
      }
      const TaskDev& T = tasks[ti];
      const ColsDev& C = cols[ti];
      if (g >= C.ngcap) continue;
      const uint4 rq = C.gmap[g];
      const u64 terr = __hip_atomic_load(&T.ctrl[2], __ATOMIC_RELAXED, __HIP_MEMORY_SCOPE_AGENT);
      const bool dead = __syncthreads_or((terr & (u64)(ERR_FALLBACK | ERR_ROWS_OVERFLOW)) != 0) != 0;
      if (rq.x == 0) continue;
      if (dead) {
        if (tid == 0) __hip_atomic_store(&C.chain[g], 2ULL << 62, __ATOMIC_RELAXED, __HIP_MEMORY_SCOPE_AGENT);
        continue;
      }
      (void)group(T, C, rq.x - 1u, rq.y, rq.z, rq.w, g);
    }
  }
#ifdef KMX_PHASE_PROF
  __syncthreads();
  if (tid == 0) for (int i = 0; i < 8; i++) atomicAdd(&kmx_sparse_prof[i], (u64)spt[i]);
#endif
}

__global__ __launch_bounds__(1024)
void k_cols_offsets(const ColsDev* __restrict__ cols, u32 task, u64* __restrict__ goff)
{
  const ColsDev& C = cols[task];
  const SpDir* dir = reinterpret_cast<const SpDir*>(C.spdir);
  __shared__ u64 part[1024];
  const u32 ng = C.slots_cap * CL_HALVES, tid = threadIdx.x;
  const u32 per = (ng + 1023) / 1024;
  u64 sum = 0;
  for (u32 g = tid * per; g < min(ng, (tid + 1) * per); g++) { sum += dir[(u64)g * CK_NPASS].dense_n; for (int p = 0; p < CK_NPASS; p++) sum += dir[(u64)g * CK_NPASS + p].n; }
  part[tid] = sum;
  __syncthreads();
  if (tid == 0) { u64 a = 0; for (u32 t = 0; t < 1024; t++) { const u64 v = part[t]; part[t] = a; a += v; } }
  __syncthreads();
  u64 a = part[tid];
  for (u32 g = tid * per; g < min(ng, (tid + 1) * per); g++) { goff[g] = a; a += dir[(u64)g * CK_NPASS].dense_n; for (int p = 0; p < CK_NPASS; p++) a += dir[(u64)g * CK_NPASS + p].n; }
}

constexpr int GA_TPB = 512;
constexpr int GA_KEYS = 4096 / KW;
template <bool COPY>
__global__ __launch_bounds__(GA_TPB)
void k_cols_gather(const TaskDev* __restrict__ tasks, const ColsDev* __restrict__ cols, u32 task, const u64* __restrict__ goff, u8* __restrict__ body)
{
  const TaskDev& T = tasks[task];
  const ColsDev& C = cols[task];
  const SpDir* dir = reinterpret_cast<const SpDir*>(C.spdir) + (u64)blockIdx.x * CK_NPASS;
  __shared__ CKey keys[GA_KEYS];
  __shared__ u32 lo[CK_NPASS + 2];
  const u32 tid = threadIdx.x, lane = tid & 63, wave = tid >> 6, row_bytes = T.row_bytes;
  if (tid == 0) { u32 a = 0; lo[0] = 0; a += dir[0].dense_n; lo[1] = a; for (int p = 0; p < CK_NPASS; p++) { a += dir[p].n; lo[2 + p] = a; } }
  __syncthreads();
  const u32 n = lo[CK_NPASS + 1];
  if (n == 0) return;
  const u32 d0 = dir[0].dense_first, dn = dir[0].dense_n;
  auto src_row = [&](u32 i) -> const u8* {
    if (i < dn) return T.out + (u64)(d0 + i) * row_bytes;
    int p = 0; while (i >= lo[2 + p]) p++;
    return T.out + (u64)(dir[p].base + (i - lo[1 + p])) * row_bytes;
  };
  auto key_at = [&](u32 i) -> CKey { return i < (u32)GA_KEYS ? keys[i] : ck_load(src_row(i)); };
  for (u32 i = tid; i < min(n, (u32)GA_KEYS); i += GA_TPB) keys[i] = i < dn ? reinterpret_cast<const CKey*>(C.skel)[d0 + i] : ck_load(src_row(i));
  __syncthreads();
  if (!COPY) {
    u32* const order = reinterpret_cast<u32*>(body) + goff[blockIdx.x];
    for (u32 i = tid; i < n; i += GA_TPB) {
      const CKey k = key_at(i);
      u32 rank = 0;
      for (int l = 0; l <= CK_NPASS; l++) {
        u32 a = lo[l], b = lo[l + 1];
        if (i >= a && i < b) { rank += i - a; continue; }
        while (a < b) { const u32 m = (a + b) >> 1; if (ck_lt(key_at(m), k)) a = m + 1; else b = m; }
        rank += a - lo[l];
      }
      order[rank] = (u32)((u64)(src_row(i) - T.out) / row_bytes);
    }
    return;
  }
  u8* const dst0 = body + goff[blockIdx.x] * row_bytes;
  __shared__ u32 rnk[GA_KEYS];
  auto rank_of = [&](u32 i) -> u32 {
    const CKey k = key_at(i);
    u32 rank = 0;
    for (int l = 0; l <= CK_NPASS; l++) {
      u32 a = lo[l], b = lo[l + 1];
      if (i >= a && i < b) { rank += i - a; continue; }
      while (a < b) { const u32 m = (a + b) >> 1; if (ck_lt(key_at(m), k)) a = m + 1; else b = m; }
      rank += a - lo[l];
    }
    return rank;
  };
  for (u32 i = tid; i < min(n, (u32)GA_KEYS); i += GA_TPB) rnk[i] = rank_of(i);
  __syncthreads();
  for (u32 i = wave; i < n; i += GA_TPB / 64) {
    const u32 rank = i < (u32)GA_KEYS ? rnk[i] : rank_of(i);
    const u8* s = src_row(i);
    u8* d = dst0 + (u64)rank * row_bytes;
    if ((row_bytes & 7u) == 0) {
      const u32 n8 = row_bytes / 8;
      for (u32 t0 = 0; t0 < n8; t0 += 512) {
        u64 w[8];
#pragma unroll
        for (int x = 0; x < 8; x++) { const u32 t = t0 + 64 * x + lane; w[x] = t < n8 ? reinterpret_cast<const u64*>(s)[t] : 0ULL; }
#pragma unroll
        for (int x = 0; x < 8; x++) { const u32 t = t0 + 64 * x + lane; if (t < n8) reinterpret_cast<u64*>(d)[t] = w[x]; }
      }
    } else if ((row_bytes & 3u) == 0) for (u32 t = lane; t < row_bytes / 4; t += 64) reinterpret_cast<u32*>(d)[t] = reinterpret_cast<const u32*>(s)[t];
    else for (u32 t = lane; t < row_bytes; t += 64) d[t] = s[t];
  }
}

void cols_dbg_dump()
{
  u32 h[16];
  if (hipMemcpyFromSymbol(h, HIP_SYMBOL(kmx_cols_dbg), sizeof(h)) != hipSuccess) return;
  if (h[9]) fprintf(stderr, "[kmx merge] k_cols_sparse: the group count of the batch was beyond every task's room (%u workgroups stopped at the room)\n", h[9]);
  if (h[8]) fprintf(stderr, "[kmx merge] k_cols_sparse: %u look-backs given up (last: group %u, %u entries still unpublished in front of it)\n", h[8], h[10], h[11]);
  fprintf(stderr, "[kmx merge] k_merge_cols hand-back reasons: no collision-free row table %u, slice overflow %u (wave-tiles; largest %u, in a range's last tile %u, first tile %u), kept key outside the row keys %u, check table full %u, lists too divergent %u (tasks)\n", h[0], h[1], h[5], h[6], h[7], h[2], h[3], h[4]);
  memset(h, 0, sizeof(h)); (void)hipMemcpyToSymbol(HIP_SYMBOL(kmx_cols_dbg), h, sizeof(h));
}
#ifdef KMX_PHASE_PROF
void cols_phase_prof_dump()
{
  u64 h[8];
  if (hipMemcpyFromSymbol(h, HIP_SYMBOL(kmx_cols_prof), sizeof(h)) != hipSuccess) return;
  u64 tot = 0; for (int i = 0; i < 8; i++) tot += h[i];
  static const char* nm[8] = {"item setup", "window wait", "scan", "bar(scan)", "tile out", "bar(out)", "-", "-"};
  for (int i = 0; i < 6; i++) fprintf(stderr, "[cols] %-12s %6.2f%%  %llu\n", nm[i], tot ? 100.0 * h[i] / tot : 0.0, h[i]);
  memset(h, 0, sizeof(h));
  (void)hipMemcpyToSymbol(HIP_SYMBOL(kmx_cols_prof), h, sizeof(h));
  if (hipMemcpyFromSymbol(h, HIP_SYMBOL(kmx_sparse_prof), sizeof(h)) != hipSuccess) return;
  tot = 0; for (int i = 0; i < 8; i++) tot += h[i];
  static const char* sn[8] = {"group entries", "zero maps", "mark twice | sample + place", "candidates | rank", "sort", "runs + claim", "rows", "gather (rec-min 1)"};
  for (int i = 0; i < 8; i++) fprintf(stderr, "[sparse] %-14s %6.2f%%  %llu\n", sn[i], tot ? 100.0 * h[i] / tot : 0.0, h[i]);
  memset(h, 0, sizeof(h));
  (void)hipMemcpyToSymbol(HIP_SYMBOL(kmx_sparse_prof), h, sizeof(h));
}
#endif

int cols_lds_bytes() { return CL_IMG + CL_NT * CL_PT * (int)sizeof(ClEnt) + 64 + 256; }
u32 cols_halves() { return CL_HALVES; }
u32 cols_wgs_per_cu() { return CL_WGS; }
u32 cols_block_lists() { return CL_NB; }
u32 cols_tile_rows(u32 nb) { return std::max(1u, std::min<u32>((u32)CL_RT, (u32)CL_IMG / (4u * std::max(1u, nb)))); }
u64 cols_scratch_keys(u32 slots, u32 nblk) { return (u64)slots * CL_HALVES * nblk * CL_NW * CL_OVW * EW; }
u64 cols_scratch_counts(u32 slots, u32 nblk) { return (u64)slots * CL_HALVES * nblk * CL_NW; }
u64 cols_ext_entries(u32 slots, u32 nblk) { return std::max<u64>(64 * 1024, (u64)slots * CL_HALVES * nblk * CL_NW * CL_OVW / 16); }

u32 cols_skel_cap() { return SK_CAP; }
hipError_t launch_cols_skel(const TaskDev* subs, const uint2* items, u32 n_items, hipStream_t st)
{
  hipLaunchKernelGGL(k_cols_skel, dim3(n_items), dim3(SK_TPB), 0, st, subs, items, n_items);
  return hipGetLastError();
}
hipError_t launch_cols_prep(const TaskDev* tasks, const TaskDev* subs, const ColsDev* cols, u32 n_tasks, hipStream_t st)
{
  hipLaunchKernelGGL(k_cols_prep, dim3(n_tasks), dim3(CP_TPB), 0, st, tasks, subs, cols);
  return hipGetLastError();
}
template <int MODE, bool EXT, bool RESC, bool ORD, bool NAR>
static hipError_t launch_merge_cols_as(const TaskDev* tasks, const ColsDev* cols, const uint2* items, u32 n_items, u32* ticket, u32 grid_x, hipStream_t st)
{
  const int lds = cols_lds_bytes();
  hipError_t e = hipFuncSetAttribute(reinterpret_cast<const void*>(&k_merge_cols<MODE, EXT, RESC, ORD, NAR>), hipFuncAttributeMaxDynamicSharedMemorySize, lds);
  if (e != hipSuccess) return e;
  hipLaunchKernelGGL((k_merge_cols<MODE, EXT, RESC, ORD, NAR>), dim3(grid_x), dim3(CL_TPB), lds, st, tasks, cols, items, n_items, ticket);
  return hipGetLastError();
}
hipError_t launch_merge_cols(int mode, int ext, const TaskDev* tasks, const ColsDev* cols, const uint2* items, u32 n_items, u32* ticket, u32 grid_x, hipStream_t st)
{
  const bool x = ext & 1, r = (ext & 2) != 0, o = (ext & 4) != 0, n = (ext & 8) != 0 && o && mode == 0;
#define KMX_CL_L3(M, X, R) (o ? launch_merge_cols_as<M, X, R, true, false>(tasks, cols, items, n_items, ticket, grid_x, st) : launch_merge_cols_as<M, X, R, false, false>(tasks, cols, items, n_items, ticket, grid_x, st))
#define KMX_CL_LAUNCH(M) (r ? (x ? KMX_CL_L3(M, true, true) : KMX_CL_L3(M, false, true)) : (x ? KMX_CL_L3(M, true, false) : KMX_CL_L3(M, false, false)))
  if (n) return r ? (x ? launch_merge_cols_as<0, true, true, true, true>(tasks, cols, items, n_items, ticket, grid_x, st) : launch_merge_cols_as<0, false, true, true, true>(tasks, cols, items, n_items, ticket, grid_x, st))
                  : (x ? launch_merge_cols_as<0, true, false, true, true>(tasks, cols, items, n_items, ticket, grid_x, st) : launch_merge_cols_as<0, false, false, true, true>(tasks, cols, items, n_items, ticket, grid_x, st));
  return mode == 0 ? KMX_CL_LAUNCH(0) : KMX_CL_LAUNCH(1);
#undef KMX_CL_L3
#undef KMX_CL_LAUNCH
}
template <int MODE, bool RESC>
static hipError_t launch_cols_sparse_ord(const TaskDev* tasks, const ColsDev* cols, u32 n_tasks, u32* ticket, u32 n_cu, hipStream_t st)
{
  static int per_cu = 0;
  if (per_cu == 0) {
    int n = 0;
    if (hipOccupancyMaxActiveBlocksPerMultiprocessor(&n, reinterpret_cast<const void*>(&k_cols_sparse<MODE, RESC, true>), ck_tpb<MODE>(), 0) != hipSuccess || n < 1) { (void)hipGetLastError(); n = 1; }
    per_cu = n;
  }
  hipLaunchKernelGGL((k_cols_sparse<MODE, RESC, true>), dim3(n_cu * (u32)per_cu), dim3(ck_tpb<MODE>()), 0, st, tasks, cols, (const uint2*)nullptr, 0u, n_tasks, ticket);
  return hipGetLastError();
}
hipError_t launch_cols_sparse(int mode, const TaskDev* tasks, const ColsDev* cols, const uint2* range_items, u32 n_items, u32 n_tasks, u32* ticket, u32 n_cu, hipStream_t st)
{
  if (mode & 4) {
    switch (mode & 3) {
      case 0: return launch_cols_sparse_ord<0, false>(tasks, cols, n_tasks, ticket, n_cu, st);
      case 1: return launch_cols_sparse_ord<1, false>(tasks, cols, n_tasks, ticket, n_cu, st);
      case 2: return launch_cols_sparse_ord<0, true>(tasks, cols, n_tasks, ticket, n_cu, st);
      default: return launch_cols_sparse_ord<1, true>(tasks, cols, n_tasks, ticket, n_cu, st);
    }
  }
  const dim3 grid(n_items, CK_Z), block(ck_tpb<0>()), block1(ck_tpb<1>());
  switch (mode & 3) {
    case 0: hipLaunchKernelGGL((k_cols_sparse<0, false, false>), grid, block, 0, st, tasks, cols, range_items, n_items, n_tasks, ticket); break;
    case 1: hipLaunchKernelGGL((k_cols_sparse<1, false, false>), grid, block1, 0, st, tasks, cols, range_items, n_items, n_tasks, ticket); break;
    case 2: hipLaunchKernelGGL((k_cols_sparse<0, true, false>), grid, block, 0, st, tasks, cols, range_items, n_items, n_tasks, ticket); break;
    default: hipLaunchKernelGGL((k_cols_sparse<1, true, false>), grid, block1, 0, st, tasks, cols, range_items, n_items, n_tasks, ticket); break;
  }
  return hipGetLastError();
}
u64 cols_dir_bytes(u32 slots) { return (u64)slots * CL_HALVES * CK_NPASS * sizeof(SpDir); }
u32 cols_groups(u32 slots) { return slots * CL_HALVES; }
hipError_t launch_cols_offsets(const ColsDev* cols, u32 task, u64* goff, hipStream_t st)
{
  hipLaunchKernelGGL(k_cols_offsets, dim3(1), dim3(1024), 0, st, cols, task, goff);
  return hipGetLastError();
}
hipError_t launch_cols_gather(const TaskDev* tasks, const ColsDev* cols, u32 task, u32 n_groups, const u64* goff, u8* body, hipStream_t st)
{
  hipLaunchKernelGGL(k_cols_gather<true>, dim3(n_groups), dim3(GA_TPB), 0, st, tasks, cols, task, goff, body);
  return hipGetLastError();
}
hipError_t launch_cols_order(const TaskDev* tasks, const ColsDev* cols, u32 task, u32 n_groups, const u64* goff, u32* order, hipStream_t st)
{
  hipLaunchKernelGGL(k_cols_gather<false>, dim3(n_groups), dim3(GA_TPB), 0, st, tasks, cols, task, goff, reinterpret_cast<u8*>(order));
  return hipGetLastError();
}

static const ColsOps g_ops = {cols_lds_bytes, cols_block_lists, cols_wgs_per_cu, cols_tile_rows, cols_scratch_keys, cols_scratch_counts, cols_ext_entries, cols_skel_cap,
                              launch_cols_skel, launch_cols_prep, launch_merge_cols, launch_cols_sparse, cols_dir_bytes, cols_groups, launch_cols_offsets,
                              launch_cols_gather, launch_cols_order, cols_dbg_dump,
#ifdef KMX_PHASE_PROF
                              cols_phase_prof_dump,
#else
                              nullptr,
#endif
                              (u32)KMX_CL_KW};
}
#if KMX_CL_KW == 1
const ColsOps& cols_ops_k1() { return cols_k1::g_ops; }
#elif KMX_CL_KW == 2
const ColsOps& cols_ops_k2() { return cols_k2::g_ops; }
#elif KMX_CL_KW == 3
const ColsOps& cols_ops_k3() { return cols_k3::g_ops; }
#else
const ColsOps& cols_ops_k4() { return cols_k4::g_ops; }
#endif
}
```

### kmtricks_amd/csrc/merge_rows.hip

```cpp
#include "kmx_dev.hpp"
#include <algorithm>
#include <cstdio>
#include <cstring>

#ifdef KMX_ROWS_SMALL
#define k_merge_rows k_merge_rows_s
#define cap_of cap_of_s
#define ts_of ts_of_s
#define rows_emit_bytes rows_emit_bytes_s
#define rows_fixed_bytes rows_fixed_bytes_s
#define rows_big rows_big_s
#define rows_lds_bytes rows_s_lds_bytes
#define rows_cap rows_s_cap
#define rows_wgs_per_cu rows_s_wgs_per_cu
#define rows_image_bytes rows_s_image_bytes
#define launch_merge_rows launch_merge_rows_s
#define kmx_phase_prof kmx_phase_prof_s
#define rows_phase_prof_dump rows_s_phase_prof_dump
#endif

namespace kmx {

#ifndef KMX_ROWS_TPB
#define KMX_ROWS_TPB 1024
#endif
#ifndef KMX_ROWS_CAP
#define KMX_ROWS_CAP 4096
#endif
constexpr int TPB = KMX_ROWS_TPB;
constexpr int CAP = KMX_ROWS_CAP;
constexpr int WGS_PER_CU = (TPB <= 512 && (CAP * 8 + 2 * CAP * 4 + CAP * 2 + 4096 + 384) * 2 <= 160 * 1024) ? 2 : 1;
constexpr int NWAVE = TPB / 64;
__host__ __device__ constexpr int cap_of(int kw, bool big = false) { return kw <= 2 || (big && kw == 3) ? CAP : (big && kw == 4) ? 3 * CAP / 4 : CAP / 2; }
__host__ __device__ constexpr int ts_of(int cap) { int t = 1; while (t < 2 * cap) t *= 2; return t; }

__host__ __device__ inline int rows_emit_bytes(int kw, bool big = false) { return cap_of(kw, big) * kw * 8; }
__host__ __device__ inline int rows_fixed_bytes(int kw, bool big = false) { return cap_of(kw, big) * kw * 8 + ts_of(cap_of(kw, big)) * 4 + cap_of(kw, big) * 2 + 4096; }

#ifndef KMX_ROWS_SMALL
template <int KW>
__global__ void k_range_bounds(const TaskDev* __restrict__ tasks, u32 max_c)
{
  const TaskDev& T = tasks[blockIdx.z];
  const u32 i = blockIdx.x * blockDim.x + threadIdx.x;
  const u32 j = blockIdx.y;
  if (i >= T.N || j > T.c) return;
  const u32 n = T.len[i];
  u32 res;
  if (j == 0) res = 0;
  else if (j == T.c) res = n;
  else {
    constexpr int RB = KW * 8 + 4;
    const u32 np = T.len[T.pivot];
    const u32 pos = (u32)(((u64)j * np) / T.c);
    const Key<KW> q = load_key<KW>(T.recs[T.pivot] + (u64)pos * RB);
    const u8* base = T.recs[i];
    u32 lo = 0, hi = n;
    if (n) {
      const u32 g = (u32)min((u64)n - 1, ((u64)pos * n) / np);
      if (key_less<KW>(load_key<KW>(base + (u64)g * RB), q)) {
        lo = g + 1;
        u32 step = 1, pr = g + 1;
        while (pr < n && key_less<KW>(load_key<KW>(base + (u64)pr * RB), q)) { lo = pr + 1; step <<= 1; pr = g + step; }
        hi = min(pr, n);
      } else {
        hi = g;
        u32 step = 1;
        while (step <= g && !key_less<KW>(load_key<KW>(base + (u64)(g - step) * RB), q)) { hi = g - step; step <<= 1; }
        lo = step <= g ? g - step + 1 : 0;
      }
    }
    while (lo < hi) {
      u32 mid = lo + ((hi - lo) >> 1);
      Key<KW> k = load_key<KW>(base + (u64)mid * RB);
      if (key_less<KW>(k, q)) lo = mid + 1; else hi = mid;
    }
    res = lo;
  }
  T.bounds[(u64)j * T.N + i] = res;
}
#endif

#ifdef KMX_PHASE_PROF
__device__ u64 kmx_phase_prof[16];
#endif

template <int KW, int TS> __device__ __forceinline__ u32 key_hash(const Key<KW>& k)
{
  u32 x = (u32)k.w[0] ^ ((u32)(k.w[0] >> 32) * 0x9E3779B1u);
  if (KW >= 2) x ^= ((u32)k.w[KW - 1] * 0x85EBCA77u) ^ ((u32)(k.w[KW - 1] >> 32) * 0xC2B2AE3Du);
  if (KW >= 3) x ^= ((u32)k.w[1] * 0x27D4EB2Fu) ^ ((u32)(k.w[1] >> 32) * 0x165667B1u);
  if (KW >= 4) x ^= ((u32)k.w[2] * 0x9E3779B1u) ^ ((u32)(k.w[2] >> 32) * 0x85EBCA77u);
  x *= 0x85EBCA6Bu; x ^= x >> 15; x *= 0x2C1B3C6Du; x ^= x >> 13;
  return x & (TS - 1);
}

__device__ __forceinline__ void lds_barrier() { asm volatile("s_waitcnt lgkmcnt(0)\n\ts_barrier" ::: "memory"); }

template <int KW, int TS>
__device__ __noinline__ u64 probe_slow(u32* tab, const Key<KW>* keysL, Key<KW> k, u32 h, u32 s)
{
  for (;;) {
    h = (h + 1) & (TS - 1);
    u32 o = tab[h];
    if (o == 0) {
      o = atomicCAS(&tab[h], 0u, s + 1);
      if (o == 0) return (u64)h;
    }
    if (key_eq<KW>(keysL[(o & 0xFFFFu) - 1], k)) return (u64)h | ((u64)o << 32);
  }
}

template <int KW, int MODE, bool BIG>
__global__ __launch_bounds__(TPB, (KW == 1 ? WGS_PER_CU : 1) * TPB / 256)
void k_merge_rows(const TaskDev* __restrict__ tasks, const uint2* __restrict__ items, u32 n_items, u32* ticket)
{
  extern __shared__ __attribute__((aligned(16))) unsigned char smem[];
  constexpr int CAP = cap_of(KW, BIG), M = CAP / TPB, TS = ts_of(CAP), KLBYTES = CAP * 2 + 4096;
  constexpr int WMIN = KW <= 2 ? 256 : NWAVE * KW * 8;
  constexpr int RB4 = (KW * 8 + 4) / 4;
  constexpr int KEYS_BYTES = CAP * KW * 8;
  constexpr int DKMAX = 4096 / (KW * 8);

  Key<KW>* keysL = reinterpret_cast<Key<KW>*>(smem);
  unsigned char* const img = smem;
  u32* tab = reinterpret_cast<u32*>(smem + KEYS_BYTES);
  u16* dslot = reinterpret_cast<u16*>(smem + KEYS_BYTES + TS * 4);
  Key<KW>* dkeys = reinterpret_cast<Key<KW>*>(smem + KEYS_BYTES + TS * 4 + CAP * 2);
  unsigned char* misc = smem + KEYS_BYTES + TS * 4 + KLBYTES;
  Key<KW>* wmin = reinterpret_cast<Key<KW>*>(misc);
  u32* wany = reinterpret_cast<u32*>(misc + WMIN);
  u64* bc64 = reinterpret_cast<u64*>(misc + WMIN + 64);
  u32* bc32 = reinterpret_cast<u32*>(misc + WMIN + 80);

  const int tid = threadIdx.x, lane = tid & 63, wave = tid >> 6;
#ifdef KMX_PHASE_PROF
  long long pt[9] = {0, 0, 0, 0, 0, 0, 0, 0, 0}; long long pc = clock64();
#define PH(i) do { const long long n_ = clock64(); pt[i] += n_ - pc; pc = n_; } while (0)
#else
#define PH(i) do {} while (0)
#endif
  {
    uint4* t4 = reinterpret_cast<uint4*>(tab);
    for (int t = tid; t < TS / 4; t += TPB) t4[t] = make_uint4(0, 0, 0, 0);
    if (tid == 0) bc32[2] = 0;
  }

  for (;;) {
    if (tid == 0) bc32[0] = atomicAdd(ticket, 1u);
    __syncthreads();
    const u32 item = (u32)__builtin_amdgcn_readfirstlane((int)bc32[0]);
    __syncthreads();
    if (item >= n_items) {
#ifdef KMX_PHASE_PROF
      if (tid == 0) for (int i = 0; i < 9; i++) atomicAdd(&kmx_phase_prof[i], (u64)pt[i]);
#endif
      return;
    }
    const TaskDev& T = tasks[items[item].x];
    const u32 range = items[item].y;
    const u32 N = T.N, wl = T.wl, w = 1u << wl;
    const u32 rec_min = T.rec_min, share_min = T.share_min, row_bytes = T.row_bytes;
    const u32 sat = max(rec_min, share_min);
    const u32 chunk_rows = max(64u, (u32)KMX_CHUNK_BYTES / row_bytes);
    const u32 g0 = lane & ~(w - 1);
    const u32 nxt = (lane + 1) & (w - 1);
    const u64 wmask = (w == 64) ? ~0ULL : ((1ULL << w) - 1);

    gu32* ptr[M]; u32 endv[M], idx[M], smin[M], nso[M]; u64 two[M];
    Key<KW> key[M]; u32 cnt[M];
    u32 lastm = 0;
#pragma unroll
    for (int m = 0; m < M; m++) {
      const u32 s = tid + m * TPB, li = s >> wl, rr = s & (w - 1);
      nso[m] = 0; two[m] = 0; idx[m] = 0; endv[m] = 0; ptr[m] = (gu32*)nullptr; smin[m] = 0;
      key[m] = key_inf<KW>(); cnt[m] = 0;
      if (li < N) {
        ptr[m] = (gu32*)(uintptr_t)T.recs[li];
        smin[m] = T.soft_min[li];
        endv[m] = T.bounds[(u64)(range + 1) * N + li];
        const u32 c0 = T.bounds[(u64)range * N + li];
        idx[m] = c0 + ((rr - c0) & (w - 1));
        if (idx[m] == c0 + w - 1) lastm |= 1u << m;
        if (idx[m] < endv[m]) {
          gu32* p = ptr[m] + (u64)idx[m] * RB4;
#pragma unroll
          for (int q = 0; q < KW; q++) key[m].w[q] = (u64)p[2 * q] | ((u64)p[2 * q + 1] << 32);
          cnt[m] = p[2 * KW];
        }
      }
    }
    u64 ch_base = 0; u32 ch_used = 0, ch_cap = 0, ch_seq = 0, ch_ok = 1;
    __syncthreads();

    u32 seq = 0;
    PH(0);
    for (;;) {
      Key<KW> cand = key_inf<KW>();
      u32 anyv = 0;
#pragma unroll
      for (int m = 0; m < M; m++) {
        anyv |= (idx[m] < endv[m]) ? 1u : 0u;
        if (((lastm >> m) & 1u) && idx[m] + 1 < endv[m]) cand = key_min<KW>(cand, key[m]);
      }
      cand = wave_min_key<KW>(cand);
      const u64 vbal = __ballot(anyv != 0);
      if (lane == 0) { wmin[wave] = cand; wany[wave] = vbal != 0; }
      lds_barrier();
      PH(1);
      Key<KW> b = wmin[0];
      u32 any = wany[0];
#pragma unroll
      for (int v = 1; v < NWAVE; v++) { b = key_min<KW>(b, wmin[v]); any |= wany[v]; }
      if (!any) break;

      Key<KW> nkey[M]; u32 ncnt[M];
      u32 consm = 0;
#pragma unroll
      for (int m = 0; m < M; m++) {
        const bool c = idx[m] < endv[m] && key_le<KW>(key[m], b);
        const u64 g = (__ballot(c) >> g0) & wmask;
        if (g && g != wmask) {
          if (c && !((g >> nxt) & 1ULL)) lastm |= 1u << m; else lastm &= ~(1u << m);
        }
        if (c) {
          consm |= 1u << m;
          keysL[tid + m * TPB] = key[m];
          const u32 ni = idx[m] + w;
          if (ni < endv[m]) {
            gu32* p = ptr[m] + (u64)ni * RB4;
#pragma unroll
            for (int q = 0; q < KW; q++) nkey[m].w[q] = (u64)p[2 * q] | ((u64)p[2 * q + 1] << 32);
            ncnt[m] = p[2 * KW];
// ... 126 lines not shown
            } else cnt[m] = 0;
          }
        }
      }
      PH(5);
      if (dk && can_write) {
        u8* const dst0 = T.out + row_off * row_bytes;
        for (u32 b0 = 0; b0 < dk; b0 += rows_per) {
          const u32 nb = min(rows_per, dk - b0);
          const u32 bytes = nb * row_bytes;
          if (b0) {
            lds_barrier();
            uint4* z = reinterpret_cast<uint4*>(img);
            for (u32 t = tid; t < (bytes + 15) / 16; t += TPB) z[t] = make_uint4(0, 0, 0, 0);
            lds_barrier();
          }
#pragma unroll
          for (int m = 0; m < M; m++) {
            const u32 r = kr[m] - b0;
            if (kr[m] != 0xFFFFu && r < nb) {
              u8* row = img + r * row_bytes;
              if ((ownm >> m) & 1u) {
                if (MODE == 0) {
                  u32* rw = reinterpret_cast<u32*>(row);
#pragma unroll
                  for (int q = 0; q < KW; q++) { rw[2 * q] = (u32)key[m].w[q]; rw[2 * q + 1] = (u32)(key[m].w[q] >> 32); }
                } else {
#pragma unroll
                  for (int q = 0; q < KW * 8; q++) row[q] = (u8)(key[m].w[q >> 3] >> ((q & 7) * 8));
                }
              }
              if (cnt[m]) {
                const u32 li = (tid + m * TPB) >> wl;
                if (MODE == 0) reinterpret_cast<u32*>(row + KW * 8)[li] = cnt[m];
                else {
                  const u32 ob = r * row_bytes + KW * 8 + (li >> 3);
                  atomicOr(reinterpret_cast<u32*>(img) + (ob >> 2), 1u << (((ob & 3u) << 3) + (li & 7u)));
                }
              }
            }
          }
          lds_barrier();
          if (b0 == 0) {
#pragma unroll
            for (int m = 0; m < M; m++) if ((ownm >> m) & 1u) tab[hs[m]] = 0;
          }
          u8* dst = dst0 + (u64)b0 * row_bytes;
          if (MODE == 0) {
            if (((reinterpret_cast<uintptr_t>(dst) | bytes) & 7u) == 0) {
              const u64* src = reinterpret_cast<const u64*>(img);
              u64* d64 = reinterpret_cast<u64*>(dst);
              for (u32 t = tid; t < bytes / 8; t += TPB) d64[t] = src[t];
            } else {
              const u32* src = reinterpret_cast<const u32*>(img);
              u32* d32 = reinterpret_cast<u32*>(dst);
              for (u32 t = tid; t < bytes / 4; t += TPB) d32[t] = src[t];
            }
          } else {
            for (u32 t = tid; t < bytes; t += TPB) dst[t] = img[t];
          }
        }
      } else {
        lds_barrier();
#pragma unroll
        for (int m = 0; m < M; m++) if ((ownm >> m) & 1u) tab[hs[m]] = 0;
      }
#pragma unroll
      for (int m = 0; m < M; m++) {
        if ((consm >> m) & 1u) {
          idx[m] += w;
          if (idx[m] < endv[m]) { key[m] = nkey[m]; cnt[m] = ncnt[m]; }
        }
      }
      PH(6);
      seq++;
    }

    if (tid == 0 && ch_used) {
      const u64 sidx = atomicAdd(&T.ctrl[1], 1ULL);
      if (sidx < T.seg_cap) { Seg sg; sg.range = range; sg.seq = ch_seq; sg.row_off = ch_base; sg.nrows = ch_used; sg.pad = 0; T.segs[sidx] = sg; }
      else atomicOr(&T.ctrl[2], (u64)ERR_SEGS_OVERFLOW);
      atomicAdd(&T.ctrl[3], (u64)ch_used);
    }
#pragma unroll
    for (int m = 0; m < M; m++) {
      u32 a = nso[m]; u64 t2 = two[m];
      for (u32 off = 1; off < w; off <<= 1) {
        a += __shfl_xor(a, (int)off); t2 += shfl_xor_u64(t2, (int)off);
      }
      const u32 s = tid + m * TPB, li = s >> wl;
      if (li < N && (s & (w - 1)) == 0 && (a | t2)) {
        if (a) atomicAdd(&T.stats[0 * (u64)N + li], (u64)a);
        atomicAdd(&T.stats[4 * (u64)N + li], t2);
      }
    }
    __syncthreads();
  }
}

#ifndef KMX_ROWS_SMALL
template __global__ void k_range_bounds<1>(const TaskDev*, u32);
template __global__ void k_range_bounds<2>(const TaskDev*, u32);
template __global__ void k_range_bounds<3>(const TaskDev*, u32);
template __global__ void k_range_bounds<4>(const TaskDev*, u32);
#endif
template __global__ void k_merge_rows<1, 0, false>(const TaskDev*, const uint2*, u32, u32*);
template __global__ void k_merge_rows<1, 1, false>(const TaskDev*, const uint2*, u32, u32*);
template __global__ void k_merge_rows<2, 0, false>(const TaskDev*, const uint2*, u32, u32*);
template __global__ void k_merge_rows<2, 1, false>(const TaskDev*, const uint2*, u32, u32*);
#ifndef KMX_ROWS_SMALL
template __global__ void k_merge_rows<3, 0, false>(const TaskDev*, const uint2*, u32, u32*);
template __global__ void k_merge_rows<3, 1, false>(const TaskDev*, const uint2*, u32, u32*);
template __global__ void k_merge_rows<4, 0, false>(const TaskDev*, const uint2*, u32, u32*);
template __global__ void k_merge_rows<4, 1, false>(const TaskDev*, const uint2*, u32, u32*);
template __global__ void k_merge_rows<3, 0, true>(const TaskDev*, const uint2*, u32, u32*);
template __global__ void k_merge_rows<3, 1, true>(const TaskDev*, const uint2*, u32, u32*);
template __global__ void k_merge_rows<4, 0, true>(const TaskDev*, const uint2*, u32, u32*);
template __global__ void k_merge_rows<4, 1, true>(const TaskDev*, const uint2*, u32, u32*);
#endif

}

namespace kmx {

static bool rows_big(int kw, u32 n) { return kw >= 3 && n > (u32)cap_of(kw); }
int rows_lds_bytes(int kw, u32 n) { return rows_fixed_bytes(kw, rows_big(kw, n)) + (kw <= 2 ? 384 : NWAVE * kw * 8 + 128); }
int rows_cap(int kw, u32 n) { return cap_of(kw, rows_big(kw, n)); }
int rows_wgs_per_cu(int kw) { return kw == 1 ? WGS_PER_CU : 1; }
#ifndef KMX_ROWS_SMALL
u32 rows_chunk_rows(u32 row_bytes) { return std::max(64u, (u32)KMX_CHUNK_BYTES / row_bytes); }
#endif
u32 rows_image_bytes(int kw) { return (u32)rows_emit_bytes(kw); }
#ifdef KMX_PHASE_PROF
void rows_phase_prof_dump()
{
  u64 h[16];
  if (hipMemcpyFromSymbol(h, HIP_SYMBOL(kmx_phase_prof), sizeof(h)) != hipSuccess) return;
  u64 tot = 0; for (int i = 0; i < 9; i++) tot += h[i];
  static const char* nm[9] = {"setup", "bound(+wait)", "consume+pref", "insert", "publish+rank", "decide", "emit+rotate", "-", "-"};
  for (int i = 0; i < 8; i++) fprintf(stderr, "[phase] %-14s %6.2f%%  %llu\n", nm[i], tot ? 100.0 * h[i] / tot : 0.0, h[i]);
  memset(h, 0, sizeof(h));
  (void)hipMemcpyToSymbol(HIP_SYMBOL(kmx_phase_prof), h, sizeof(h));
}
#endif

#ifndef KMX_ROWS_SMALL
hipError_t launch_range_bounds(int kw, const TaskDev* tasks, u32 n_tasks, u32 max_n, u32 max_c, hipStream_t st)
{
  dim3 grid((max_n + 255) / 256, max_c + 1, n_tasks), block(256);
  if (kw == 1) hipLaunchKernelGGL(k_range_bounds<1>, grid, block, 0, st, tasks, max_c);
  else if (kw == 2) hipLaunchKernelGGL(k_range_bounds<2>, grid, block, 0, st, tasks, max_c);
  else if (kw == 3) hipLaunchKernelGGL(k_range_bounds<3>, grid, block, 0, st, tasks, max_c);
  else hipLaunchKernelGGL(k_range_bounds<4>, grid, block, 0, st, tasks, max_c);
  return hipGetLastError();
}
#endif

hipError_t launch_merge_rows(int kw, int mode, const TaskDev* tasks, const uint2* items, u32 n_items, u32* ticket,
                             u32 grid_x, u32 max_n, hipStream_t st)
{
  const int lds = rows_lds_bytes(kw, max_n);
  dim3 grid(grid_x), block(TPB);
#define KMX_LAUNCH(KW_, MODE_, BIG_)                                                                              \
  do {                                                                                                      \
    hipError_t e_ = hipFuncSetAttribute(reinterpret_cast<const void*>(&k_merge_rows<KW_, MODE_, BIG_>),           \
                                        hipFuncAttributeMaxDynamicSharedMemorySize, lds);                   \
    if (e_ != hipSuccess) return e_;                                                                        \
    hipLaunchKernelGGL((k_merge_rows<KW_, MODE_, BIG_>), grid, block, lds, st, tasks, items, n_items, ticket);    \
  } while (0)
  if (kw == 1 && mode == 0) KMX_LAUNCH(1, 0, false);
  else if (kw == 1 && mode == 1) KMX_LAUNCH(1, 1, false);
  else if (kw == 2 && mode == 0) KMX_LAUNCH(2, 0, false);
  else if (kw == 2 && mode == 1) KMX_LAUNCH(2, 1, false);
#ifndef KMX_ROWS_SMALL
  else if (kw == 3 && mode == 0 && rows_big(3, max_n)) KMX_LAUNCH(3, 0, true);
  else if (kw == 3 && mode == 1 && rows_big(3, max_n)) KMX_LAUNCH(3, 1, true);
  else if (kw == 4 && mode == 0 && rows_big(4, max_n)) KMX_LAUNCH(4, 0, true);
  else if (kw == 4 && mode == 1 && rows_big(4, max_n)) KMX_LAUNCH(4, 1, true);
  else if (kw == 3 && mode == 0) KMX_LAUNCH(3, 0, false);
  else if (kw == 3 && mode == 1) KMX_LAUNCH(3, 1, false);
  else if (kw == 4 && mode == 0) KMX_LAUNCH(4, 0, false);
  else if (kw == 4 && mode == 1) KMX_LAUNCH(4, 1, false);
#endif
  else return hipErrorInvalidValue;
#undef KMX_LAUNCH
  return hipGetLastError();
}

}
```

### kmtricks_amd/lib.py

```python
import ctypes as C
import os
import numpy as np

_HERE = os.path.dirname(os.path.abspath(__file__))
LIB_PATH = os.environ.get("KMX_LIB") or os.path.join(_HERE, "libkmx.so")
if not os.path.exists(LIB_PATH):
    raise ImportError(f"{LIB_PATH} is missing: build it with `python -c 'import __graft_entry__ as g; g.build()'` "
                      "(libkmx has no CPU fallback)")
_lib = C.CDLL(LIB_PATH)

MODE_COUNT, MODE_PA, MODE_BF, MODE_BFC, MODE_BFT = 0, 1, 2, 3, 4
STATS_ROWS = 6


class KmxList(C.Structure):
    _fields_ = [("recs", C.c_void_p), ("n", C.c_uint64)]


class KmxMergeTask(C.Structure):
    _fields_ = [("n_lists", C.c_uint32), ("key_words", C.c_uint32), ("lists", C.POINTER(KmxList)),
                ("soft_min", C.POINTER(C.c_uint32)), ("rec_min", C.c_uint32), ("share_min", C.c_uint32),
                ("mode", C.c_uint32), ("bitw", C.c_uint32), ("lower", C.c_uint64), ("upper", C.c_uint64),
                ("rows_hint", C.c_uint64), ("list_on_device", C.c_void_p)]

# ... 139 lines not shown
_lib.kmx_peer_access.argtypes = [C.c_int, C.c_int]
EXPORTS = ["kmx_copy_to_host_async", "kmx_copy_wait", "kmx_reads_upload", "kmx_reads_release", "kmx_peer_access", "kmx_set_file_order", "kmx_count_reads_dev_multi", "kmx_version", "kmx_result_prepare_body", "kmx_result_arena", "kmx_result_copy_order", "kmx_result_sparse_rows", "kmx_device_memory", "kmx_superk_sample", "kmx_store_create", "kmx_store_destroy", "kmx_store_used", "kmx_store_limit", "kmx_copy_to_host", "kmx_count_reads_dev", "kmx_hist_reset", "kmx_hist_read", "kmx_hist_off", "kmx_device_count", "kmx_count_reads", "kmx_result_copy_body_dev", "kmx_merge_host", "kmx_alloc_pinned", "kmx_free_pinned", "kmx_superk_partition_stats", "kmx_result_transpose_ms", "kmx_result_body_dev", "kmx_set_profiling", "kmx_result_kernel_ms", "kmx_result_kernel", "kmx_create", "kmx_destroy", "kmx_last_error", "kmx_stream", "kmx_merge_dev",
           "kmx_result_wait", "kmx_result_rows", "kmx_result_row_bytes", "kmx_result_body_bytes",
           "kmx_result_algo_bytes", "kmx_result_copy_body", "kmx_result_copy_stats", "kmx_result_free",
           "kmx_merge", "kmx_count_kmer", "kmx_count_hash", "kmx_count_batch", "kmx_transpose_bits", "kmx_superk_partition",
           "kmx_free"]

_lib.kmx_filter_dev.argtypes = [_vp, C.POINTER(KmxFilterTask), C.POINTER(_vp)]
_lib.kmx_filter_host.argtypes = [_vp, C.POINTER(KmxFilterTask), C.POINTER(_vp)]
_lib.kmx_filter_result_wait.argtypes = [_vp]
for _f in ("kmx_filter_result_rows", "kmx_filter_result_row_bytes", "kmx_filter_result_body_bytes", "kmx_filter_result_vector_len",
           "kmx_filter_result_absent", "kmx_filter_result_algo_bytes"):
    getattr(_lib, _f).restype = C.c_uint64
    getattr(_lib, _f).argtypes = [_vp]
for _f in ("kmx_filter_result_body_dev", "kmx_filter_result_vector_dev", "kmx_filter_result_absent_dev"):
    getattr(_lib, _f).restype = _vp
    getattr(_lib, _f).argtypes = [_vp]
for _f in ("kmx_filter_result_copy_body", "kmx_filter_result_copy_vector", "kmx_filter_result_copy_absent"):
    getattr(_lib, _f).argtypes = [_vp, _vp, C.c_uint64]
_lib.kmx_filter_result_kernel_ms.restype = C.c_double
_lib.kmx_filter_result_kernel_ms.argtypes = [_vp]
_lib.kmx_filter_result_free.argtypes = [_vp]
_lib.kmx_filter_marks_alloc.restype = _vp
_lib.kmx_filter_marks_alloc.argtypes = [_vp, C.c_uint64]
_lib.kmx_filter_marks_free.argtypes = [_vp, _vp]


_lib.kmx_combine_dev.argtypes = [_vp, C.POINTER(KmxCombineTask), C.POINTER(_vp)]
_lib.kmx_combine_host.argtypes = [_vp, C.POINTER(KmxCombineTask), C.POINTER(_vp)]
_lib.kmx_combine_result_wait.argtypes = [_vp]
for _f in ("kmx_combine_result_rows", "kmx_combine_result_row_bytes", "kmx_combine_result_body_bytes", "kmx_combine_result_algo_bytes"):
    getattr(_lib, _f).restype = C.c_uint64
    getattr(_lib, _f).argtypes = [_vp]
_lib.kmx_combine_result_body_dev.restype = _vp
_lib.kmx_combine_result_body_dev.argtypes = [_vp]
_lib.kmx_combine_result_copy_body.argtypes = [_vp, _vp, C.c_uint64]
_lib.kmx_combine_result_kernel_ms.restype = C.c_double
_lib.kmx_combine_result_kernel_ms.argtypes = [_vp]
_lib.kmx_combine_result_free.argtypes = [_vp]

_lib.kmx_query_dev.argtypes = [_vp, C.POINTER(KmxQueryTask), C.POINTER(_vp)]
_lib.kmx_query_host.argtypes = [_vp, C.POINTER(KmxQueryTask), C.POINTER(_vp)]
_lib.kmx_query_result_wait.argtypes = [_vp]
for _f in ("kmx_query_result_n_seqs", "kmx_query_result_algo_bytes"):
    getattr(_lib, _f).restype = C.c_uint64
    getattr(_lib, _f).argtypes = [_vp]
for _f in ("kmx_query_result_copy_kmers", "kmx_query_result_copy_hits"):
    getattr(_lib, _f).argtypes = [_vp, _vp, C.c_uint64]
_lib.kmx_query_result_hits_dev.restype = _vp
_lib.kmx_query_result_hits_dev.argtypes = [_vp]
_lib.kmx_query_result_kernel_ms.restype = C.c_double
_lib.kmx_query_result_kernel_ms.argtypes = [_vp]
_lib.kmx_query_result_free.argtypes = [_vp]

_lib.kmx_kquery_dev.argtypes = [_vp, C.POINTER(KmxKqueryTask), C.POINTER(_vp)]
_lib.kmx_kquery_host.argtypes = [_vp, C.POINTER(KmxKqueryTask), C.POINTER(_vp)]
_lib.kmx_kquery_result_wait.argtypes = [_vp]
for _f in ("kmx_kquery_result_n_seqs", "kmx_kquery_result_algo_bytes"):
    getattr(_lib, _f).restype = C.c_uint64
    getattr(_lib, _f).argtypes = [_vp]
for _f in ("kmx_kquery_result_copy_kmers", "kmx_kquery_result_copy_hits", "kmx_kquery_result_copy_sums"):
    getattr(_lib, _f).argtypes = [_vp, _vp, C.c_uint64]
for _f in ("kmx_kquery_result_hits_dev", "kmx_kquery_result_sums_dev"):
    getattr(_lib, _f).restype = _vp
    getattr(_lib, _f).argtypes = [_vp]
_lib.kmx_kquery_result_kernel_ms.restype = C.c_double
_lib.kmx_kquery_result_kernel_ms.argtypes = [_vp]
_lib.kmx_kquery_result_free.argtypes = [_vp]
KQUERY_EXPORTS = ["kmx_kquery_dev", "kmx_kquery_host", "kmx_kquery_result_wait", "kmx_kquery_result_n_seqs", "kmx_kquery_result_copy_kmers",
                  "kmx_kquery_result_copy_hits", "kmx_kquery_result_copy_sums", "kmx_kquery_result_hits_dev", "kmx_kquery_result_sums_dev",
                  "kmx_kquery_result_kernel_ms", "kmx_kquery_result_algo_bytes", "kmx_kquery_result_free"]

_lib.kmx_zquery_bits_bytes.restype = C.c_uint64
_lib.kmx_zquery_bits_bytes.argtypes = [C.c_uint64, C.c_uint32]
_lib.kmx_zquery_dev.argtypes = [_vp, C.POINTER(KmxZqueryTask), C.POINTER(_vp)]
_lib.kmx_zquery_host.argtypes = [_vp, C.POINTER(KmxZqueryTask), C.POINTER(_vp)]
_lib.kmx_zquery_result_wait.argtypes = [_vp]
for _f in ("kmx_zquery_result_n_seqs", "kmx_zquery_result_algo_bytes"):
    getattr(_lib, _f).restype = C.c_uint64
    getattr(_lib, _f).argtypes = [_vp]
for _f in ("kmx_zquery_result_copy_kmers", "kmx_zquery_result_copy_hits"):
    getattr(_lib, _f).argtypes = [_vp, _vp, C.c_uint64]
for _f in ("kmx_zquery_result_hits_dev", "kmx_zquery_result_bits_dev"):
    getattr(_lib, _f).restype = _vp
    getattr(_lib, _f).argtypes = [_vp]
_lib.kmx_zquery_result_kernel_ms.restype = C.c_double
_lib.kmx_zquery_result_kernel_ms.argtypes = [_vp]
_lib.kmx_zquery_result_free.argtypes = [_vp]
ZQUERY_EXPORTS = ["kmx_zquery_bits_bytes", "kmx_zquery_dev", "kmx_zquery_host", "kmx_zquery_result_wait", "kmx_zquery_result_n_seqs",
                  "kmx_zquery_result_copy_kmers", "kmx_zquery_result_copy_hits", "kmx_zquery_result_hits_dev", "kmx_zquery_result_bits_dev",
                  "kmx_zquery_result_kernel_ms", "kmx_zquery_result_algo_bytes", "kmx_zquery_result_free"]


def zquery_bits_bytes(n_bases, n_cols):
    return _lib.kmx_zquery_bits_bytes(n_bases, n_cols)


def filter_want(want):
    if isinstance(want, int):
        return want
    bits = {"m": FILTER_M, "v": FILTER_V, "k": FILTER_K}
    return sum({bits[c] for c in want.replace(",", "")})


def key_words_of(k):
    return (k + 31) // 32


class KmxError(RuntimeError):
    pass


def pack_records(keys, counts, key_words=1):
    keys = np.ascontiguousarray(keys, dtype=np.uint64).reshape(-1, key_words)
    counts = np.ascontiguousarray(counts, dtype=np.uint32)
    n = len(counts)
    rec = np.zeros((n, key_words * 2 + 1), dtype=np.uint32)
    rec[:, :key_words * 2] = keys.view(np.uint32).reshape(n, key_words * 2)
    rec[:, key_words * 2] = counts
    return rec


class Context:

    def __init__(self, device=0):
        h = _vp()
        rc = _lib.kmx_create(device, C.byref(h))
        if rc != 0:
            raise KmxError(f"kmx_create failed ({rc}): {_lib.kmx_last_error(None).decode()}")
        self._h = h
        self.device = device

    def close(self):
        if self._h:
            _lib.kmx_destroy(self._h)
            self._h = None

    def __del__(self):
        try:
            self.close()
        except Exception:
            pass

    def _check(self, rc, what):
        if rc != 0:
            raise KmxError(f"{what} failed ({rc}): {_lib.kmx_last_error(self._h).decode()}")

    def set_profiling(self, on=True):
        self._check(_lib.kmx_set_profiling(self._h, 1 if on else 0), "kmx_set_profiling")

    def set_file_order(self, on=True):
        self._check(_lib.kmx_set_file_order(self._h, 1 if on else 0), "kmx_set_file_order")

    @property
    def stream(self):
        return _lib.kmx_stream(self._h)

    @staticmethod
    def _task(lists_ptr_n, key_words, soft_min, rec_min, share_min, mode, lower, upper, bitw, rows_hint, keep):
        n = len(lists_ptr_n)
        arr = (KmxList * n)()
        for i, (p, cnt) in enumerate(lists_ptr_n):
            arr[i].recs = p
            arr[i].n = cnt
        sm = (C.c_uint32 * n)(*[int(x) for x in soft_min])
        keep.extend([arr, sm])
        t = KmxMergeTask()
        t.n_lists, t.key_words, t.lists, t.soft_min = n, key_words, arr, sm
        t.rec_min, t.share_min, t.mode, t.bitw = rec_min, share_min, mode, bitw
        t.lower, t.upper, t.rows_hint = lower, upper, rows_hint
        return t

    def merge(self, lists, key_words, soft_min, rec_min, share_min, mode, lower=0, upper=0, bitw=2, rows_hint=0):
        keep, recs = [], []
        for k, c in lists:
            r = pack_records(k, c, key_words)
            recs.append(r)
        t = self._task([(r.ctypes.data if len(r) else None, len(r)) for r in recs], key_words, soft_min, rec_min,
                       share_min, mode, lower, upper, bitw, rows_hint, keep)
        body, nb, rows = _vp(), C.c_uint64(), C.c_uint64()
        stats = np.zeros((STATS_ROWS, len(lists)), dtype=np.uint64)
        self._check(_lib.kmx_merge(self._h, C.byref(t), C.byref(body), C.byref(nb), C.byref(rows), stats.ctypes.data),
                    "kmx_merge")
        data = (C.string_at(body.value, nb.value) if nb.value < (1 << 31) else bytes((C.c_ubyte * nb.value).from_address(body.value))) if nb.value else b""
        _lib.kmx_free(body)
        return data, rows.value, stats

    def _take(self, kp, cp, n, width):
        keys = np.ctypeslib.as_array((C.c_uint64 * (n * width)).from_address(kp.value)).copy().reshape(n, width) if n \
            else np.zeros((0, width), np.uint64)
        cnts = np.ctypeslib.as_array((C.c_uint32 * n).from_address(cp.value)).copy() if n else np.zeros(0, np.uint32)
        _lib.kmx_free(kp)
        _lib.kmx_free(cp)
        return keys, cnts

    def count_kmer(self, superk: bytes, k, hard_min):
        kp, cp, n = _vp(), _vp(), C.c_uint64()
        self._check(_lib.kmx_count_kmer(self._h, superk, len(superk), k, hard_min, C.byref(kp), C.byref(cp),
                                        C.byref(n)), "kmx_count_kmer")
        return self._take(kp, cp, n.value, key_words_of(k))

    def count_hash(self, superk: bytes, k, window, partition, hard_min):
        kp, cp, n = _vp(), _vp(), C.c_uint64()
        self._check(_lib.kmx_count_hash(self._h, superk, len(superk), k, window, partition, hard_min, C.byref(kp),
                                        C.byref(cp), C.byref(n)), "kmx_count_hash")
        keys, cnts = self._take(kp, cp, n.value, 1)
        return keys.reshape(-1), cnts

    def count_batch(self, streams, k, hard_min, window=0, partitions=None):
        n = len(streams)
        sp = (C.c_char_p * n)(*[s if s else None for s in streams])
        ln = (C.c_uint64 * n)(*[len(s) for s in streams])
        pid = (C.c_uint64 * n)(*(partitions if partitions is not None else range(n)))
        kp, cp, no = (_vp * n)(), (_vp * n)(), (C.c_uint64 * n)()
        self._check(_lib.kmx_count_batch(self._h, n, sp, ln, k, 1 if window else 0, window, pid, hard_min, kp, cp, no),
                    "kmx_count_batch")
        width = 1 if window else key_words_of(k)
        out = []
        for p in range(n):
            keys, cnts = self._take(_vp(kp[p]), _vp(cp[p]), no[p], width)
            out.append((keys.reshape(-1) if window else keys, cnts))
        return out

    def transpose_bits(self, mat, nrows, ncols):
        mat = np.ascontiguousarray(mat, dtype=np.uint8)
        out = np.zeros(ncols * (nrows // 8), dtype=np.uint8)
        self._check(_lib.kmx_transpose_bits(self._h, mat.ctypes.data, nrows, ncols, out.ctypes.data),
                    "kmx_transpose_bits")
        return out

    @staticmethod
    def pack_reads(reads):
        bs = [r if isinstance(r, bytes) else r.encode() for r in reads]
        offs = np.zeros(len(bs) + 1, dtype=np.uint64)
        offs[1:] = np.cumsum([len(b) for b in bs], dtype=np.uint64)
        return b"".join(bs), offs

    def superk_partition(self, reads, k, m, repart, nb_parts):
        blob, offs = reads if isinstance(reads, tuple) else self.pack_reads(reads)
        rep = np.ascontiguousarray(repart, dtype=np.uint16)
        ob = (_vp * nb_parts)()
        ol = (C.c_uint64 * nb_parts)()
        okm = (C.c_uint64 * nb_parts)()
        self._check(_lib.kmx_superk_partition(self._h, blob, offs.ctypes.data, len(offs) - 1, k, m, rep.ctypes.data, nb_parts,
                                              ob, ol, okm), "kmx_superk_partition")
        out = []
        for p in range(nb_parts):
            out.append((C.string_at(ob[p], ol[p]) if ol[p] else b"", int(okm[p])))
            _lib.kmx_free(ob[p])
        return out

    def superk_partition_stats(self, reads, k, m, repart, nb_parts, streams=True):
        blob, offs = reads if isinstance(reads, tuple) else self.pack_reads(reads)
        rep = np.ascontiguousarray(repart, dtype=np.uint16)
        pin = np.zeros(nb_parts * PINFO_STRIDE, dtype=np.uint64)
        ms, mk, mx = (np.zeros(4 ** m, dtype=np.uint64) for _ in range(3))
        st = KmxSuperkStats(pin.ctypes.data, ms.ctypes.data, mk.ctypes.data, mx.ctypes.data, 0)
        ob = (_vp * nb_parts)()
        ol = (C.c_uint64 * nb_parts)()
        okm = (C.c_uint64 * nb_parts)()
        self._check(_lib.kmx_superk_partition_stats(self._h, blob, offs.ctypes.data, len(offs) - 1, k, m, rep.ctypes.data,
                                                    nb_parts, ob if streams else None, ol, okm, C.byref(st)),
                    "kmx_superk_partition_stats")
        out = None
        if streams:
            out = []
            for p in range(nb_parts):
                out.append((C.string_at(ob[p], ol[p]) if ol[p] else b"", int(okm[p])))
                _lib.kmx_free(ob[p])
        assert st.nb_superk == int(ms.sum())
        return out, pin.reshape(nb_parts, -1), ms, mk, mx

    def count_reads(self, reads, k, m, repart, nb_parts, hard_min, window=0, streams=False):
        blob, offs = reads if isinstance(reads, tuple) else self.pack_reads(reads)
        rep = np.ascontiguousarray(repart, dtype=np.uint16)
        kp, cp, no, nk = (_vp * nb_parts)(), (_vp * nb_parts)(), (C.c_uint64 * nb_parts)(), (C.c_uint64 * nb_parts)()
        ob, ol = (_vp * nb_parts)(), (C.c_uint64 * nb_parts)()
        info = (C.c_uint64 * (2 * nb_parts))()
        self._check(_lib.kmx_count_reads(self._h, blob, offs.ctypes.data, len(offs) - 1, k, m, rep.ctypes.data, nb_parts,
                                         1 if window else 0, window, hard_min, kp, cp, no, nk, ob if streams else None,
                                         ol if streams else None, info, None), "kmx_count_reads")
        width = 1 if window else key_words_of(k)
        out = []
        for p in range(nb_parts):
            keys, cnts = self._take(_vp(kp[p]), _vp(cp[p]), no[p], width)
            out.append((keys.reshape(-1) if window else keys, cnts))
        st = None
        if streams:
            st = []
            for p in range(nb_parts):
                st.append(C.string_at(ob[p], ol[p]) if ol[p] else b"")
                _lib.kmx_free(ob[p])
        return out, [int(x) for x in nk], st, np.array(list(info), dtype=np.uint64).reshape(nb_parts, 2)

    def upload_reads(self, blob, offs=None):
        n = len(blob)
        at = (n + 63) & ~63
        nb = 0 if offs is None else 8 * len(offs)
        pin = _lib.kmx_alloc_pinned(max(at + nb, 1))
        C.memmove(pin, blob, n)
        po = None
        if offs is not None:
            po = np.frombuffer((C.c_char * nb).from_address(pin + at), dtype=np.uint64)
            po[:] = np.ascontiguousarray(offs, dtype=np.uint64)
        dev = _vp()
        self._check(_lib.kmx_reads_upload(self._h, pin, n, C.byref(dev)), "kmx_reads_upload")
# ... 674 lines not shown
```

Baseline: 128.2 billion.

## Fuse cols skeleton and prep into the merge kernel front with ready flags

By default the columnar path now merges the two range-bounds launches into one kernel. It also runs the skeleton and prep work as a persistent front phase inside k_merge_cols, whose workgroups grab front items by ticket. The last skeleton workgroup of each task runs prep and publishes a ready flag, and merge items spin-wait on that flag. This removes several kernel launches and inter-kernel serialization, at the cost of spin-waits, memory fences, and a fallback when the flag never arrives. A debug counter readout API is also added.

```diff
diff --git a/include/kmx.h b/include/kmx.h
--- a/include/kmx.h
+++ b/include/kmx.h
@@ -68,6 +68,7 @@
 int      kmx_result_wait(kmx_merge_result* r);
 double   kmx_result_kernel_ms(kmx_merge_result* r);
 int      kmx_result_kernel_parts_ms(kmx_merge_result* r, double* first_ms, double* second_ms);
+int      kmx_cols_debug_counters(kmx_ctx* ctx, uint32_t key_words, uint32_t out[16]);
 const char* kmx_result_kernel(const kmx_merge_result* r);
 double   kmx_result_transpose_ms(kmx_merge_result* r);
 const void* kmx_result_body_dev(kmx_merge_result* r, uint32_t task);
diff --git a/kmtricks_amd/csrc/kmx_api.hip b/kmtricks_amd/csrc/kmx_api.hip
--- a/kmtricks_amd/csrc/kmx_api.hip
+++ b/kmtricks_amd/csrc/kmx_api.hip
@@ -402,6 +402,14 @@
 }
 
 extern "C" int kmx_set_profiling(kmx_ctx* ctx, int on) { if (!ctx) return KMX_E_INVAL; ctx->profiling = on != 0; return KMX_OK; }
+extern "C" int kmx_cols_debug_counters(kmx_ctx* ctx, uint32_t key_words, uint32_t out[16])
+{
+  if (!ctx) return KMX_E_INVAL;
+  if (!out || key_words < 1 || key_words > 2) return ctx->fail(KMX_E_INVAL, "kmx_cols_debug_counters: key_words must be 1 or 2, out not null");
+  KMX_HIP(ctx, hipSetDevice(ctx->device));
+  cols_ops((int)key_words).dbg_read(out);
+  return KMX_OK;
+}
 extern "C" int kmx_set_file_order(kmx_ctx* ctx, int on) { if (!ctx) return KMX_E_INVAL; ctx->file_order = on != 0; return KMX_OK; }
 
 struct TaskHost {
@@ -540,6 +548,13 @@
     const ColsDev* d_cols = reinterpret_cast<const ColsDev*>(R->d_meta + R->o_cols);
     const uint2* d_citems = reinterpret_cast<const uint2*>(R->d_meta + R->o_citems);
     static const bool overlap = getenv("KMX_COLS_PREP_OVERLAP") != nullptr;
+    static const bool front = !overlap && !(getenv("KMX_COLS_FRONT") && getenv("KMX_COLS_FRONT")[0] == '0');
+    const u32 cols_grid_env = getenv("KMX_COLS_GRID") ? (u32)atoi(getenv("KMX_COLS_GRID")) : 0u;
+    const u32 sparse_cus_env = getenv("KMX_SPARSE_CUS") ? (u32)atoi(getenv("KMX_SPARSE_CUS")) : 0u;
+    if (front) {
+      KMX_HIP(ctx, hipStreamWaitEvent(ctx->stream, R->ev_up, 0));
+      KMX_HIP(ctx, launch_range_bounds2(kw, d_tasks, R->max_n, R->max_c, d_subs, R->sub_max_n, R->sub_max_c, nt, ctx->stream));
+    } else {
     hipStream_t ps = overlap ? ctx->aux : ctx->stream;
     if (!R->ev_pre) KMX_HIP(ctx, hipEventCreateWithFlags(&R->ev_pre, hipEventDisableTiming));
     if (overlap && ctx->stream_shared) {
@@ -554,11 +569,10 @@
     KMX_HIP(ctx, hipStreamWaitEvent(ctx->stream, R->ev_up, 0));
     KMX_HIP(ctx, launch_range_bounds(kw, d_tasks, nt, R->max_n, R->max_c, ctx->stream));
     KMX_HIP(ctx, hipStreamWaitEvent(ctx->stream, R->ev_pre, 0));
+    }
     if (R->ev0) KMX_HIP(ctx, hipEventRecord(R->ev0, ctx->stream));
-    const u32 cols_grid_env = getenv("KMX_COLS_GRID") ? (u32)atoi(getenv("KMX_COLS_GRID")) : 0u;
-    const u32 sparse_cus_env = getenv("KMX_SPARSE_CUS") ? (u32)atoi(getenv("KMX_SPARSE_CUS")) : 0u;
     KMX_HIP(ctx, CO.merge(mode, (R->cols_ext ? 1 : 0) | (R->cols_resc ? 2 : 0) | (R->cols_ord ? 4 : 0) | (R->cols_narrow ? 8 : 0), d_tasks, d_cols, d_citems, R->n_citems, d_ticket,
-                          cols_grid_env ? std::min(cols_grid_env, R->cols_grid) : R->cols_grid, ctx->stream));
+                          cols_grid_env ? std::min(cols_grid_env, R->cols_grid) : R->cols_grid, ctx->stream, d_subs, d_subitems, front ? R->n_subitems : 0u));
     if (R->ev0) { if (!R->ev_mid) KMX_HIP(ctx, hipEventCreate(&R->ev_mid)); KMX_HIP(ctx, hipEventRecord(R->ev_mid, ctx->stream)); }
     KMX_HIP(ctx, CO.sparse(mode | (R->cols_resc ? 2 : 0) | (R->cols_ord ? 4 : 0), d_tasks, d_cols, d_items, R->n_items, nt, d_ticket, sparse_cus_env ? std::min(sparse_cus_env, (u32)ctx->n_cu) : (u32)ctx->n_cu, ctx->stream));
     if (R->share_fix) {
diff --git a/kmtricks_amd/csrc/kmx_host.hpp b/kmtricks_amd/csrc/kmx_host.hpp
--- a/kmtricks_amd/csrc/kmx_host.hpp
+++ b/kmtricks_amd/csrc/kmx_host.hpp
@@ -15,6 +15,7 @@
 u32 rows_chunk_rows(u32 row_bytes);
 u32 rows_image_bytes(int kw);
 hipError_t launch_range_bounds(int kw, const TaskDev* tasks, u32 n_tasks, u32 max_n, u32 max_c, hipStream_t st);
+hipError_t launch_range_bounds2(int kw, const TaskDev* tasks_a, u32 max_n_a, u32 max_c_a, const TaskDev* tasks_b, u32 max_n_b, u32 max_c_b, u32 n_tasks, hipStream_t st);
 hipError_t launch_merge_rows(int kw, int mode, const TaskDev* tasks, const uint2* items, u32 n_items, u32* ticket,
                              u32 grid_x, u32 max_n, hipStream_t st);
 int rows_s_cap(int kw, u32 n_lists);
@@ -36,7 +37,8 @@
   u32 (*skel_cap)();
   hipError_t (*skel)(const TaskDev* subs, const uint2* items, u32 n_items, hipStream_t st);
   hipError_t (*prep)(const TaskDev* tasks, const TaskDev* subs, const ColsDev* cols, u32 n_tasks, hipStream_t st);
-  hipError_t (*merge)(int mode, int ext, const TaskDev* tasks, const ColsDev* cols, const uint2* items, u32 n_items, u32* ticket, u32 grid_x, hipStream_t st);
+  hipError_t (*merge)(int mode, int ext, const TaskDev* tasks, const ColsDev* cols, const uint2* items, u32 n_items, u32* ticket, u32 grid_x, hipStream_t st,
+                      const TaskDev* subs, const uint2* front_items, u32 n_front_items);
   hipError_t (*sparse)(int mode, const TaskDev* tasks, const ColsDev* cols, const uint2* range_items, u32 n_items, u32 n_tasks, u32* ticket, u32 n_cu, hipStream_t st);
   u64 (*dir_bytes)(u32 slots);
   u32 (*groups)(u32 slots);
@@ -44,6 +46,7 @@
   hipError_t (*gather)(const TaskDev* tasks, const ColsDev* cols, u32 task, u32 n_groups, const u64* goff, u8* body, hipStream_t st);
   hipError_t (*order)(const TaskDev* tasks, const ColsDev* cols, u32 task, u32 n_groups, const u64* goff, u32* order, hipStream_t st);
   void (*dbg_dump)();
+  void (*dbg_read)(u32* out16);
   void (*phase_prof_dump)();
   u32 key_words;
 };
diff --git a/kmtricks_amd/csrc/merge_cols.hip b/kmtricks_amd/csrc/merge_cols.hip
--- a/kmtricks_amd/csrc/merge_cols.hip
+++ b/kmtricks_amd/csrc/merge_cols.hip
@@ -162,25 +162,25 @@
 #endif
 constexpr int SK_TPB = KMX_SK_TPB;
 constexpr int SK_CAP = 2048;
-
-__global__ __launch_bounds__(SK_TPB)
-void k_cols_skel(const TaskDev* __restrict__ subs, const uint2* __restrict__ items, u32 n_items)
-{
-  __shared__ CKey ks[SK_CAP];
-  __shared__ u32 wsum[SK_TPB / 64];
-  const u32 item = blockIdx.x;
-  if (item >= n_items) return;
-  const TaskDev& S = subs[items[item].x];
-  const u32 range = items[item].y, N = S.N, rec_min = max(1u, S.rec_min);
+constexpr int SK_KS_BYTES = SK_CAP * (int)sizeof(CKey);
+constexpr int SK_LDS = SK_KS_BYTES + 128;
+
+template <int TPB>
+__device__ __forceinline__ void cols_skel_range(const TaskDev& S, const u32 range, unsigned char* lds)
+{
+  CKey* const ks = reinterpret_cast<CKey*>(lds);
+  u32* const wsum = reinterpret_cast<u32*>(lds + SK_KS_BYTES);
+  u32& irregular = *reinterpret_cast<u32*>(lds + SK_KS_BYTES + 64);
+  constexpr u32 SK_TPB = TPB;
+  const u32 N = S.N, rec_min = max(1u, S.rec_min);
   const u32 tid = threadIdx.x, lane = tid & 63, wave = tid >> 6;
   u32 total = 0;
   for (u32 i = 0; i < N; i++) total += S.bounds[(u64)(range + 1) * N + i] - S.bounds[(u64)range * N + i];
   Seg sg; sg.range = range; sg.seq = 0; sg.row_off = (u64)range * SK_CAP; sg.nrows = 0; sg.pad = 0;
   if (total > (u32)SK_CAP) {
-    if (tid == 0) { atomicOr(&S.ctrl[2], (u64)ERR_ROWS_OVERFLOW); S.segs[range] = sg; atomicAdd(&S.ctrl[1], 1ULL); }
+    if (tid == 0) { atomicOr(&S.ctrl[2], (u64)ERR_ROWS_OVERFLOW); S.segs[range] = sg; }
     return;
   }
-  __shared__ u32 irregular;
   u32 maxn = 1;
   for (u32 i = 0; i < N; i++) maxn = max(maxn, S.bounds[(u64)(range + 1) * N + i] - S.bounds[(u64)range * N + i]);
   u32 L = 1; while (L < maxn) L <<= 1;
@@ -250,27 +250,39 @@
   for (u32 w = 0; w < SK_TPB / 64; w++) { if (w < wave) base += wsum[w]; nk += wsum[w]; }
   CKey* out = reinterpret_cast<CKey*>(S.out) + (u64)range * SK_CAP;
   for (u32 x = 0; x < per; x++) if ((keptm >> x) & 1u) out[base++] = ks[tid * per + x];
-  if (tid == 0) { sg.nrows = nk; S.segs[range] = sg; atomicAdd(&S.ctrl[1], 1ULL); atomicAdd(&S.ctrl[3], (u64)nk); }
+  if (tid == 0) { sg.nrows = nk; S.segs[range] = sg; atomicAdd(&S.ctrl[3], (u64)nk); }
+}
+
+__global__ __launch_bounds__(SK_TPB)
+void k_cols_skel(const TaskDev* __restrict__ subs, const uint2* __restrict__ items, u32 n_items)
+{
+  __shared__ __attribute__((aligned(16))) unsigned char lds[SK_LDS];
+  const u32 item = blockIdx.x;
+  if (item >= n_items) return;
+  const TaskDev& S = subs[items[item].x];
+  cols_skel_range<SK_TPB>(S, items[item].y, lds);
+  if (threadIdx.x == 0) atomicAdd(&S.ctrl[1], 1ULL);
 }
 
 constexpr int CP_TPB = 1024;
-__global__ __launch_bounds__(CP_TPB)
-void k_cols_prep(const TaskDev* __restrict__ tasks, const TaskDev* __restrict__ subs, const ColsDev* __restrict__ cols)
-{
-  const TaskDev& T = tasks[blockIdx.x];
-  const TaskDev& S = subs[blockIdx.x];
-  const ColsDev& C = cols[blockIdx.x];
-  __shared__ u32 s_off[CP_MAXSEG];
-  __shared__ u64 s_ord[CP_MAXSEG];
-  __shared__ u32 s_n[CP_MAXSEG];
+constexpr int CP_LDS = CP_MAXSEG * 16 + 16;
+template <int TPB>
+__device__ __forceinline__ void cols_prep_task(const TaskDev& T, const TaskDev& S, const ColsDev& C, unsigned char* lds)
+{
+  u64* const s_ord = reinterpret_cast<u64*>(lds);
+  u32* const s_off = reinterpret_cast<u32*>(lds + CP_MAXSEG * 8);
+  u32* const s_n = reinterpret_cast<u32*>(lds + CP_MAXSEG * 12);
+  u32& s_ng = *reinterpret_cast<u32*>(lds + CP_MAXSEG * 16);
+  constexpr u32 CP_TPB = TPB;
   const u32 tid = threadIdx.x;
-  const u64 serr = S.ctrl[2], nseg64 = S.ctrl[1], rows = S.ctrl[3];
+  const u64 serr = __hip_atomic_load(&S.ctrl[2], __ATOMIC_RELAXED, __HIP_MEMORY_SCOPE_AGENT), nseg64 = __hip_atomic_load(&S.ctrl[1], __ATOMIC_RELAXED, __HIP_MEMORY_SCOPE_AGENT),
+            rows = __hip_atomic_load(&S.ctrl[3], __ATOMIC_RELAXED, __HIP_MEMORY_SCOPE_AGENT);
   if (tid == 0) T.ctrl[7] = rows;
   const u64 slots = rows / C.rt + T.c + 2;
   const bool dense_small = C.dense != nullptr && rows > (u64)C.dense_cap;
   const bool bad = serr != 0 || nseg64 > (u64)CP_MAXSEG || nseg64 > S.seg_cap || rows > T.out_cap_rows || rows > 0xFFFFFF00ULL ||
                    slots > C.slots_cap || dense_small;
-  const u64 nsolid = S.ctrl[4], ncov = S.ctrl[5];
+  const u64 nsolid = __hip_atomic_load(&S.ctrl[4], __ATOMIC_RELAXED, __HIP_MEMORY_SCOPE_AGENT), ncov = __hip_atomic_load(&S.ctrl[5], __ATOMIC_RELAXED, __HIP_MEMORY_SCOPE_AGENT);
   const bool divergent = (nsolid - ncov) * 8 > nsolid;
   if (divergent && !bad) {
     if (tid == 0) { atomicOr(&T.ctrl[2], (u64)(ERR_FALLBACK | ERR_DIVERGENT)); *C.nskel = 0; atomicAdd(&kmx_cols_dbg[4], 1u); }
@@ -321,7 +333,6 @@
     T.segs[0] = sg;
   }
   if (C.gbase) {
-    __shared__ u32 s_ng;
     __syncthreads();
     if (tid == 0) {
       u32 g = 0;
@@ -339,6 +350,13 @@
   }
 }
 
+__global__ __launch_bounds__(CP_TPB)
+void k_cols_prep(const TaskDev* __restrict__ tasks, const TaskDev* __restrict__ subs, const ColsDev* __restrict__ cols)
+{
+  __shared__ __attribute__((aligned(16))) unsigned char lds[CP_LDS];
+  cols_prep_task<CP_TPB>(tasks[blockIdx.x], subs[blockIdx.x], cols[blockIdx.x], lds);
+}
+
 __device__ const u32 kmx_cols_sentinel[8] = {~0u, ~0u, KW == 1 ? 0u : ~0u, KW == 1 ? 0u : ~0u, 0u, 0u, 0u, 0u};
 
 #ifdef KMX_PHASE_PROF
@@ -350,10 +368,55 @@
 #endif
 
 constexpr u64 CL_NONSOLID = 1ULL << 63;
+constexpr int CF_READY = 6;
+constexpr u32 CF_READY_SPINS = 1u << 20;
+constexpr int CF_SH = SK_LDS > CP_LDS ? SK_LDS : CP_LDS;
+constexpr int CF_LDS = CF_SH + 16;
+__device__ __forceinline__ void cf_release_all()
+{
+  asm volatile("s_waitcnt vmcnt(0)" ::: "memory");
+  __syncthreads();
+  if (threadIdx.x == 0) { __builtin_amdgcn_fence(__ATOMIC_RELEASE, "agent"); asm volatile("s_waitcnt vmcnt(0)" ::: "memory"); }
+}
+template <int TPB>
+__device__ __forceinline__ void cols_front(const TaskDev* __restrict__ tasks, const TaskDev* __restrict__ subs, const ColsDev* __restrict__ cols,
+                                           const uint2* __restrict__ fitems, const u32 n_fitems, u32* fticket, unsigned char* lds)
+{
+  u32* const fsh = reinterpret_cast<u32*>(lds + CF_SH);
+  for (;;) {
+    if (threadIdx.x == 0) fsh[0] = atomicAdd(fticket, 1u);
+    __syncthreads();
+    const u32 item = cl_uni(fsh[0]);
+    __syncthreads();
+    if (item >= n_fitems) return;
+    const u32 t = cl_uni(fitems[item].x);
+    const TaskDev& S = subs[t];
+    cols_skel_range<TPB>(S, cl_uni(fitems[item].y), lds);
+    cf_release_all();
+    if (threadIdx.x == 0) fsh[1] = atomicAdd(&S.ctrl[1], 1ULL) + 1ULL == (u64)S.c ? 1u : 0u;
+    __syncthreads();
+    if (cl_uni(fsh[1])) {
+      __builtin_amdgcn_fence(__ATOMIC_ACQUIRE, "agent");
+      cols_prep_task<TPB>(tasks[t], S, cols[t], lds);
+      cf_release_all();
+      if (threadIdx.x == 0) __hip_atomic_store(&S.ctrl[CF_READY], 1ULL, __ATOMIC_RELAXED, __HIP_MEMORY_SCOPE_AGENT);
+    }
+    __syncthreads();
+  }
+}
+__device__ __forceinline__ bool cf_wait_ready(const u64* w)
+{
+  for (u32 spins = 0; __hip_atomic_load(w, __ATOMIC_RELAXED, __HIP_MEMORY_SCOPE_AGENT) == 0; ) {
+    __builtin_amdgcn_s_sleep(8);
+    if (++spins > CF_READY_SPINS) return false;
+  }
+  return true;
+}
+
 template <int MODE, bool EXT, bool RESC, bool ORD, bool NAR>
 __global__ __launch_bounds__(CL_TPB, CL_WGS)
 void k_merge_cols(const TaskDev* __restrict__ tasks, const ColsDev* __restrict__ cols, const uint2* __restrict__ items,
-                  u32 n_items, u32* ticket)
+                  u32 n_items, u32* ticket, const TaskDev* __restrict__ subs, const uint2* __restrict__ fitems, u32 n_fitems)
 {
   extern __shared__ __attribute__((aligned(16))) unsigned char smem[];
   u32* const img = reinterpret_cast<u32*>(smem);
@@ -363,15 +426,17 @@
 
   const int tid = threadIdx.x, lane = tid & 63;
   const u32 wave = cl_uni((u32)tid >> 6);
-  for (int t = tid; t < CL_IMG / 16; t += CL_TPB) reinterpret_cast<uint4*>(img)[t] = make_uint4(0, 0, 0, 0);
-  for (int t = tid; t < CL_NT * CL_PT; t += CL_TPB) ptab[t].idx = 0;
-  if (tid == 0) { sh[1] = 0; sh[2] = 0; sh[3] = 0; }
 #ifdef KMX_PHASE_PROF
   long long pt[8] = {0, 0, 0, 0, 0, 0, 0, 0}; long long pc = clock64();
 #define CLPH(i) do { const long long n_ = clock64(); pt[i] += n_ - pc; pc = n_; } while (0)
 #else
 #define CLPH(i) do {} while (0)
 #endif
+  static_assert(CF_LDS <= CL_IMG + CL_NT * CL_PT * (int)sizeof(ClEnt), "the front's LDS lies in the tile image and the row tables");
+  if (n_fitems) { cols_front<CL_TPB>(tasks, subs, cols, fitems, n_fitems, ticket + 4, smem); CLPH(6); }
+  for (int t = tid; t < CL_IMG / 16; t += CL_TPB) reinterpret_cast<uint4*>(img)[t] = make_uint4(0, 0, 0, 0);
+  for (int t = tid; t < CL_NT * CL_PT; t += CL_TPB) ptab[t].idx = 0;
+  if (tid == 0) { sh[1] = 0; sh[2] = 0; sh[3] = 0; }
 
   for (;;) {
     if (tid == 0) sh[0] = atomicAdd(ticket, 1u);
@@ -386,6 +451,14 @@
     }
     const TaskDev& T = tasks[items[item].x];
     const ColsDev& C = cols[items[item].x];
+    if (n_fitems) {
+      const int there = __syncthreads_or(tid == 0 ? (int)cf_wait_ready(&subs[items[item].x].ctrl[CF_READY]) : 0);
+      __builtin_amdgcn_fence(__ATOMIC_ACQUIRE, "agent");
+      if (!there) {
+        if (tid == 0) { atomicOr(&T.ctrl[2], (u64)ERR_FALLBACK); atomicAdd(&kmx_cols_dbg[13], 1u); }
+        continue;
+      }
+    }
     if (__syncthreads_or((__hip_atomic_load(&T.ctrl[2], __ATOMIC_RELAXED, __HIP_MEMORY_SCOPE_AGENT) & (u64)(ERR_FALLBACK | ERR_ROWS_OVERFLOW)) != 0)) continue;
     const u32 N = cl_uni(T.N), row_bytes = cl_uni(T.row_bytes), nblk = cl_uni(C.nblk), nbs = cl_uni(C.nb), rt = cl_uni(C.rt);
     const u32 range = cl_uni(items[item].y) / nblk, blk = cl_uni(items[item].y) - range * nblk;
@@ -1608,11 +1681,16 @@
   }
 }
 
+void cols_dbg_read(u32* out16)
+{
+  if (hipMemcpyFromSymbol(out16, HIP_SYMBOL(kmx_cols_dbg), 16 * sizeof(u32)) != hipSuccess) { (void)hipGetLastError(); for (int i = 0; i < 16; i++) out16[i] = ~0u; }
+}
 void cols_dbg_dump()
 {
   u32 h[16];
   if (hipMemcpyFromSymbol(h, HIP_SYMBOL(kmx_cols_dbg), sizeof(h)) != hipSuccess) return;
   if (h[9]) fprintf(stderr, "[kmx merge] k_cols_sparse: the group count of the batch was beyond every task's room (%u workgroups stopped at the room)\n", h[9]);
+  if (h[13]) fprintf(stderr, "[kmx merge] k_merge_cols: %u merge items dropped, their task's row keys never came\n", h[13]);
   if (h[8]) fprintf(stderr, "[kmx merge] k_cols_sparse: %u look-backs given up (last: group %u, %u entries still unpublished in front of it)\n", h[8], h[10], h[11]);
   fprintf(stderr, "[kmx merge] k_merge_cols hand-back reasons: no collision-free row table %u, slice overflow %u (wave-tiles; largest %u, in a range's last tile %u, first tile %u), kept key outside the row keys %u, check table full %u, lists too divergent %u (tasks)\n", h[0], h[1], h[5], h[6], h[7], h[2], h[3], h[4]);
   memset(h, 0, sizeof(h)); (void)hipMemcpyToSymbol(HIP_SYMBOL(kmx_cols_dbg), h, sizeof(h));
@@ -1623,8 +1701,8 @@
   u64 h[8];
   if (hipMemcpyFromSymbol(h, HIP_SYMBOL(kmx_cols_prof), sizeof(h)) != hipSuccess) return;
   u64 tot = 0; for (int i = 0; i < 8; i++) tot += h[i];
-  static const char* nm[8] = {"item setup", "window wait", "scan", "bar(scan)", "tile out", "bar(out)", "-", "-"};
-  for (int i = 0; i < 6; i++) fprintf(stderr, "[cols] %-12s %6.2f%%  %llu\n", nm[i], tot ? 100.0 * h[i] / tot : 0.0, h[i]);
+  static const char* nm[8] = {"item setup", "window wait", "scan", "bar(scan)", "tile out", "bar(out)", "front", "-"};
+  for (int i = 0; i < 7; i++) fprintf(stderr, "[cols] %-12s %6.2f%%  %llu\n", nm[i], tot ? 100.0 * h[i] / tot : 0.0, h[i]);
   memset(h, 0, sizeof(h));
   (void)hipMemcpyToSymbol(HIP_SYMBOL(kmx_cols_prof), h, sizeof(h));
   if (hipMemcpyFromSymbol(h, HIP_SYMBOL(kmx_sparse_prof), sizeof(h)) != hipSuccess) return;
@@ -1657,21 +1735,23 @@
   return hipGetLastError();
 }
 template <int MODE, bool EXT, bool RESC, bool ORD, bool NAR>
-static hipError_t launch_merge_cols_as(const TaskDev* tasks, const ColsDev* cols, const uint2* items, u32 n_items, u32* ticket, u32 grid_x, hipStream_t st)
+static hipError_t launch_merge_cols_as(const TaskDev* tasks, const ColsDev* cols, const uint2* items, u32 n_items, u32* ticket, u32 grid_x, hipStream_t st,
+                                       const TaskDev* subs, const uint2* fitems, u32 n_fitems)
 {
   const int lds = cols_lds_bytes();
   hipError_t e = hipFuncSetAttribute(reinterpret_cast<const void*>(&k_merge_cols<MODE, EXT, RESC, ORD, NAR>), hipFuncAttributeMaxDynamicSharedMemorySize, lds);
   if (e != hipSuccess) return e;
-  hipLaunchKernelGGL((k_merge_cols<MODE, EXT, RESC, ORD, NAR>), dim3(grid_x), dim3(CL_TPB), lds, st, tasks, cols, items, n_items, ticket);
+  hipLaunchKernelGGL((k_merge_cols<MODE, EXT, RESC, ORD, NAR>), dim3(grid_x), dim3(CL_TPB), lds, st, tasks, cols, items, n_items, ticket, subs, fitems, n_fitems);
   return hipGetLastError();
 }
-hipError_t launch_merge_cols(int mode, int ext, const TaskDev* tasks, const ColsDev* cols, const uint2* items, u32 n_items, u32* ticket, u32 grid_x, hipStream_t st)
+hipError_t launch_merge_cols(int mode, int ext, const TaskDev* tasks, const ColsDev* cols, const uint2* items, u32 n_items, u32* ticket, u32 grid_x, hipStream_t st,
+                             const TaskDev* subs, const uint2* fitems, u32 n_fitems)
 {
   const bool x = ext & 1, r = (ext & 2) != 0, o = (ext & 4) != 0, n = (ext & 8) != 0 && o && mode == 0;
-#define KMX_CL_L3(M, X, R) (o ? launch_merge_cols_as<M, X, R, true, false>(tasks, cols, items, n_items, ticket, grid_x, st) : launch_merge_cols_as<M, X, R, false, false>(tasks, cols, items, n_items, ticket, grid_x, st))
+#define KMX_CL_L3(M, X, R) (o ? launch_merge_cols_as<M, X, R, true, false>(tasks, cols, items, n_items, ticket, grid_x, st, subs, fitems, n_fitems) : launch_merge_cols_as<M, X, R, false, false>(tasks, cols, items, n_items, ticket, grid_x, st, subs, fitems, n_fitems))
 #define KMX_CL_LAUNCH(M) (r ? (x ? KMX_CL_L3(M, true, true) : KMX_CL_L3(M, false, true)) : (x ? KMX_CL_L3(M, true, false) : KMX_CL_L3(M, false, false)))
-  if (n) return r ? (x ? launch_merge_cols_as<0, true, true, true, true>(tasks, cols, items, n_items, ticket, grid_x, st) : launch_merge_cols_as<0, false, true, true, true>(tasks, cols, items, n_items, ticket, grid_x, st))
-                  : (x ? launch_merge_cols_as<0, true, false, true, true>(tasks, cols, items, n_items, ticket, grid_x, st) : launch_merge_cols_as<0, false, false, true, true>(tasks, cols, items, n_items, ticket, grid_x, st));
+  if (n) return r ? (x ? launch_merge_cols_as<0, true, true, true, true>(tasks, cols, items, n_items, ticket, grid_x, st, subs, fitems, n_fitems) : launch_merge_cols_as<0, false, true, true, true>(tasks, cols, items, n_items, ticket, grid_x, st, subs, fitems, n_fitems))
+                  : (x ? launch_merge_cols_as<0, true, false, true, true>(tasks, cols, items, n_items, ticket, grid_x, st, subs, fitems, n_fitems) : launch_merge_cols_as<0, false, false, true, true>(tasks, cols, items, n_items, ticket, grid_x, st, subs, fitems, n_fitems));
   return mode == 0 ? KMX_CL_LAUNCH(0) : KMX_CL_LAUNCH(1);
 #undef KMX_CL_L3
 #undef KMX_CL_LAUNCH
@@ -1727,7 +1807,7 @@
 
 static const ColsOps g_ops = {cols_lds_bytes, cols_block_lists, cols_wgs_per_cu, cols_tile_rows, cols_scratch_keys, cols_scratch_counts, cols_ext_entries, cols_skel_cap,
                               launch_cols_skel, launch_cols_prep, launch_merge_cols, launch_cols_sparse, cols_dir_bytes, cols_groups, launch_cols_offsets,
-                              launch_cols_gather, launch_cols_order, cols_dbg_dump,
+                              launch_cols_gather, launch_cols_order, cols_dbg_dump, cols_dbg_read,
 #ifdef KMX_PHASE_PROF
                               cols_phase_prof_dump,
 #else
diff --git a/kmtricks_amd/csrc/merge_rows.hip b/kmtricks_amd/csrc/merge_rows.hip
--- a/kmtricks_amd/csrc/merge_rows.hip
+++ b/kmtricks_amd/csrc/merge_rows.hip
@@ -39,11 +39,8 @@
 
 #ifndef KMX_ROWS_SMALL
 template <int KW>
-__global__ void k_range_bounds(const TaskDev* __restrict__ tasks, u32 max_c)
-{
-  const TaskDev& T = tasks[blockIdx.z];
-  const u32 i = blockIdx.x * blockDim.x + threadIdx.x;
-  const u32 j = blockIdx.y;
+__device__ __forceinline__ void range_bound(const TaskDev& T, const u32 i, const u32 j)
+{
   if (i >= T.N || j > T.c) return;
   const u32 n = T.len[i];
   u32 res;
@@ -79,6 +76,23 @@
   }
   T.bounds[(u64)j * T.N + i] = res;
 }
+template <int KW>
+__global__ void k_range_bounds(const TaskDev* __restrict__ tasks, u32 max_c)
+{
+  range_bound<KW>(tasks[blockIdx.z], blockIdx.x * blockDim.x + threadIdx.x, blockIdx.y);
+}
+template <int KW>
+__global__ void k_range_bounds2(const TaskDev* __restrict__ ta, u32 gx_a, u32 gy_a, const TaskDev* __restrict__ tb, u32 gx_b, u32 gy_b, u32 n)
+{
+  u32 b = blockIdx.x;
+  const u32 na = gx_a * gy_a * n;
+  const bool second = b >= na;
+  if (second) b -= na;
+  const u32 gx = second ? gx_b : gx_a, gy = second ? gy_b : gy_a;
+  const u32 t = b / (gx * gy), r = b - t * (gx * gy);
+  if (t >= n) return;
+  range_bound<KW>((second ? tb : ta)[t], (r % gx) * blockDim.x + threadIdx.x, r / gx);
+}
 #endif
 
 #ifdef KMX_PHASE_PROF
@@ -511,6 +525,21 @@
   else if (kw == 2) hipLaunchKernelGGL(k_range_bounds<2>, grid, block, 0, st, tasks, max_c);
   else if (kw == 3) hipLaunchKernelGGL(k_range_bounds<3>, grid, block, 0, st, tasks, max_c);
   else hipLaunchKernelGGL(k_range_bounds<4>, grid, block, 0, st, tasks, max_c);
+  return hipGetLastError();
+}
+hipError_t launch_range_bounds2(int kw, const TaskDev* tasks_a, u32 max_n_a, u32 max_c_a, const TaskDev* tasks_b, u32 max_n_b, u32 max_c_b, u32 n_tasks, hipStream_t st)
+{
+  const u32 gx_a = (max_n_a + 255) / 256, gy_a = max_c_a + 1, gx_b = (max_n_b + 255) / 256, gy_b = max_c_b + 1;
+  const unsigned long long nblocks = ((unsigned long long)gx_a * gy_a + (unsigned long long)gx_b * gy_b) * n_tasks;
+  if (nblocks > 0x7FFFFFFFULL) {
+    const hipError_t e = launch_range_bounds(kw, tasks_a, n_tasks, max_n_a, max_c_a, st);
+    return e != hipSuccess ? e : launch_range_bounds(kw, tasks_b, n_tasks, max_n_b, max_c_b, st);
+  }
+  const dim3 grid((unsigned)nblocks), block(256);
+  if (kw == 1) hipLaunchKernelGGL(k_range_bounds2<1>, grid, block, 0, st, tasks_a, gx_a, gy_a, tasks_b, gx_b, gy_b, n_tasks);
+  else if (kw == 2) hipLaunchKernelGGL(k_range_bounds2<2>, grid, block, 0, st, tasks_a, gx_a, gy_a, tasks_b, gx_b, gy_b, n_tasks);
+  else if (kw == 3) hipLaunchKernelGGL(k_range_bounds2<3>, grid, block, 0, st, tasks_a, gx_a, gy_a, tasks_b, gx_b, gy_b, n_tasks);
+  else hipLaunchKernelGGL(k_range_bounds2<4>, grid, block, 0, st, tasks_a, gx_a, gy_a, tasks_b, gx_b, gy_b, n_tasks);
   return hipGetLastError();
 }
 #endif
diff --git a/kmtricks_amd/lib.py b/kmtricks_amd/lib.py
--- a/kmtricks_amd/lib.py
+++ b/kmtricks_amd/lib.py
@@ -315,6 +315,12 @@
     def set_file_order(self, on=True):
         self._check(_lib.kmx_set_file_order(self._h, 1 if on else 0), "kmx_set_file_order")
 
+    def cols_debug_counters(self, key_words=1):
+        out = (C.c_uint32 * 16)()
+        _lib.kmx_cols_debug_counters.argtypes = [_vp, C.c_uint32, C.POINTER(C.c_uint32)]
+        self._check(_lib.kmx_cols_debug_counters(self._h, key_words, out), "kmx_cols_debug_counters")
+        return [int(v) for v in out]
+
     @property
     def stream(self):
         return _lib.kmx_stream(self._h)
```

Result: slower. 122.6 billion (-4.4%).
